# lab-incert/peba1

Hardware: AMD Instinct MI355X
Metric: bootstrapped gates/sec (blind rotations/s) over the PEBA1 match path, and end-to-end match ms (higher is better)
Workload: dtype u32

## Files before the change

### include/tfhe_hip.h

```cpp
#ifndef TFHE_HIP_H
#define TFHE_HIP_H

#include <stdio.h>

#include "tfhe/tfhe_core.h"

#ifdef __cplusplus
extern "C" {
#endif

enum TfheHipGate {
    TFHE_HIP_NAND = 0, TFHE_HIP_OR, TFHE_HIP_AND, TFHE_HIP_NOR, TFHE_HIP_XOR, TFHE_HIP_XNOR,
    TFHE_HIP_ANDNY, TFHE_HIP_ANDYN, TFHE_HIP_ORNY, TFHE_HIP_ORYN
};

const char *tfhe_hip_last_error(void);
void tfhe_hip_clear_error(void);

int tfhe_hip_set_device(int device);
int tfhe_hip_get_device(void);
int tfhe_hip_device_pci_bus_id(char *out, int len);

TFheGateBootstrappingParameterSet *tfhe_hip_new_parameters(
    int32_t n, int32_t N, int32_t k, int32_t l, int32_t Bgbit, int32_t ks_t, int32_t ks_basebit,
    double ks_stdev, double bk_stdev, double max_stdev);
TFheGateBootstrappingParameterSet *tfhe_hip_new_p2048_parameters(void);

TFheGateBootstrappingSecretKeySet *tfhe_hip_new_secret_keyset_seeded(
    const TFheGateBootstrappingParameterSet *params, uint64_t seed);
TFheGateBootstrappingSecretKeySet *tfhe_hip_new_secret_keyset_seeded_host(
    const TFheGateBootstrappingParameterSet *params, uint64_t seed);
void tfhe_hip_set_encrypt_seed(uint64_t seed);
int tfhe_hip_randomness_is_seeded(void);
void tfhe_hip_test_chacha20_block(const uint32_t *key8, uint64_t counter, const uint32_t *nonce2, uint32_t *out16);

const int32_t *tfhe_hip_key_lwe(const TFheGateBootstrappingSecretKeySet *key, int64_t *count);
const int32_t *tfhe_hip_key_tlwe(const TFheGateBootstrappingSecretKeySet *key, int64_t *count);
const Torus32 *tfhe_hip_key_bk(const TFheGateBootstrappingCloudKeySet *cloud, int64_t *count);
const Torus32 *tfhe_hip_key_ksk(const TFheGateBootstrappingCloudKeySet *cloud, int64_t *count);

int32_t tfhe_hip_sample_words(const TFheGateBootstrappingParameterSet *params);
int tfhe_hip_export_samples(const LweSample *samples, int32_t count,
                            const TFheGateBootstrappingParameterSet *params, Torus32 *out_words);
int tfhe_hip_import_samples(LweSample *samples, int32_t count,
                            const TFheGateBootstrappingParameterSet *params, const Torus32 *in_words);
int tfhe_hip_export_samples_device(const LweSample *samples, int32_t count,
                                   const TFheGateBootstrappingParameterSet *params, void *device_words);
int tfhe_hip_import_samples_device(LweSample *samples, int32_t count,
                                   const TFheGateBootstrappingParameterSet *params, const void *device_words);
int tfhe_hip_export_samples_device_async(const LweSample *samples, int32_t count,
                                         const TFheGateBootstrappingParameterSet *params, void *device_words);
int tfhe_hip_import_samples_device_async(LweSample *samples, int32_t count,
                                         const TFheGateBootstrappingParameterSet *params, const void *device_words);
void *tfhe_hip_stream(void);
int tfhe_hip_sync_samples(const LweSample *samples, int32_t count);

void tfhe_hip_set_deferred(int on);
int tfhe_hip_get_deferred(void);
int tfhe_hip_flush(void);
int tfhe_hip_flush_async(void);
int tfhe_hip_wait(void);

#define TFHE_HIP_EXIT_DEADLINE 86
int tfhe_hip_stream_sync(void);
int tfhe_hip_wait_event(void *hip_event, const char *what);
void tfhe_hip_set_diag_label(const char *label);

int tfhe_hip_gate_batch(int gate, LweSample *result, const LweSample *a, const LweSample *b,
                        int32_t count, const TFheGateBootstrappingCloudKeySet *bk);

enum TfheHipGate3 { TFHE_HIP_MAJ3 = 0, TFHE_HIP_XOR3, TFHE_HIP_XNOR3 };
void tfhe_hip_gate3(int gate, int negate_mask, LweSample *result, const LweSample *a, const LweSample *b,
                    const LweSample *c, const TFheGateBootstrappingCloudKeySet *bk);
int tfhe_hip_gate3_batch(int gate, int negate_mask, LweSample *result, const LweSample *a, const LweSample *b,
                         const LweSample *c, int32_t count, const TFheGateBootstrappingCloudKeySet *bk);

typedef struct TfheHipLut TfheHipLut;
TfheHipLut *tfhe_hip_new_lut(const TFheGateBootstrappingParameterSet *params, const Torus32 *v);
TfheHipLut *tfhe_hip_new_lut_constant(const TFheGateBootstrappingParameterSet *params, Torus32 mu);
TfheHipLut *tfhe_hip_new_lut_from_table(const TFheGateBootstrappingParameterSet *params, const Torus32 *values, int32_t slots);
void tfhe_hip_delete_lut(TfheHipLut *lut);
const Torus32 *tfhe_hip_lut_words(const TfheHipLut *lut, int32_t *count);
void tfhe_hip_lut_bootstrap(const TfheHipLut *lut, LweSample *result, int32_t nin, const LweSample *const *in,
                            const int32_t *coef, Torus32 c0, const TFheGateBootstrappingCloudKeySet *bk);
int tfhe_hip_lut_bootstrap_batch(const TfheHipLut *lut, LweSample *result, int32_t nin, const LweSample *const *in,
                                 const int32_t *coef, Torus32 c0, int32_t count, const TFheGateBootstrappingCloudKeySet *bk);

typedef struct TfheHipLutMulti TfheHipLutMulti;
TfheHipLutMulti *tfhe_hip_new_lut_multi(const TfheHipLut *lut, int32_t nout, const int32_t *ntaps, const int32_t *tap_index,
                                        const int32_t *tap_weight, const Torus32 *out_c0);
TfheHipLutMulti *tfhe_hip_new_lut_multi_from_tables(const TFheGateBootstrappingParameterSet *params, Torus32 step, int32_t slots,
                                                    int32_t nout, const int32_t *levels );
void tfhe_hip_delete_lut_multi(TfheHipLutMulti *mo);
int32_t tfhe_hip_lut_multi_nout(const TfheHipLutMulti *mo);
int32_t tfhe_hip_lut_multi_output(const TfheHipLutMulti *mo, int32_t m, int32_t *tap_index, int32_t *tap_weight, Torus32 *out_c0);
const Torus32 *tfhe_hip_lut_multi_words(const TfheHipLutMulti *mo, int32_t *count);
void tfhe_hip_lut_bootstrap_multi(const TfheHipLutMulti *mo, LweSample *const *result , int32_t nin,
                                  const LweSample *const *in, const int32_t *coef, Torus32 c0,
                                  const TFheGateBootstrappingCloudKeySet *bk);
int tfhe_hip_lut_bootstrap_multi_batch(const TfheHipLutMulti *mo, LweSample *const *result , int32_t nin,
                                       const LweSample *const *in, const int32_t *coef, Torus32 c0, int32_t count,
                                       const TFheGateBootstrappingCloudKeySet *bk);

#define TFHE_HIP_LINEAR_MAX_IN 16
void tfhe_hip_linear(LweSample *result, int32_t nin, const LweSample *const *in, const int32_t *coef, Torus32 c0,
                     const TFheGateBootstrappingCloudKeySet *bk);
int tfhe_hip_linear_batch(LweSample *result, int32_t nin, const LweSample *const *in, const int32_t *coef, Torus32 c0,
                          int32_t count, const TFheGateBootstrappingCloudKeySet *bk);
void tfhe_hip_sym_encrypt_torus(LweSample *result, Torus32 mu, const TFheGateBootstrappingSecretKeySet *key);
Torus32 tfhe_hip_sym_phase(const LweSample *sample, const TFheGateBootstrappingSecretKeySet *key);

int tfhe_hip_set_tuning(const char *name, int64_t value);

typedef struct TfheHipStats {
    uint64_t blind_rotates;
    uint64_t keyswitches;
    uint64_t linear_ops;
    uint64_t levels;
    uint64_t flushes;
    uint64_t br_launches;
    double   ms_blind_rotate;
    double   ms_keyswitch;
    double   ms_flush_wall;
    double   ms_blind_rotate_busy;
    uint64_t reused_gates;
    uint64_t br8_launches;
    uint64_t br8_rotations;
    double   ms_blind_rotate8;
    uint64_t clk_shader_cycles;
    uint64_t clk_ref_ticks;
    uint64_t dead_gates;
    uint64_t folded_gates;
    uint64_t br_wide4_launches;
    uint64_t br_split_launches;
    uint64_t br_wave8_launches;
    uint64_t br_wave2_launches;
    uint64_t br_tables0_launches;
    uint64_t br_tables1_launches;
    uint64_t br_tables2_launches;
    uint64_t lut_rotations;
    uint64_t multi_rotations;
    uint64_t multi_outputs;
    uint64_t lincomb_ops;
    uint64_t lincomb_launches;
    uint64_t ks_pergate_launches;
    uint64_t ks_strip_launches;
    uint64_t ks_index_launches;
    uint64_t unpacked_samples;
    uint64_t unpack_launches;
} TfheHipStats;
void tfhe_hip_get_stats(TfheHipStats *out);
void tfhe_hip_reset_stats(void);
typedef struct TfheHipExpandStats {
    uint64_t expanded_keys;
    uint64_t expand_launches;
} TfheHipExpandStats;
void tfhe_hip_get_expand_stats(TfheHipExpandStats *out);
typedef struct TfheHipSeededStats {
    uint64_t expanded_packing_keys;
    uint64_t packing_expand_launches;
    uint64_t seeded_unpacked_samples;
    uint64_t seeded_unpack_launches;
} TfheHipSeededStats;
void tfhe_hip_get_seeded_stats(TfheHipSeededStats *out);
typedef struct TfheHipSeededLweStats {
    uint64_t seeded_imported_samples;
    uint64_t seeded_import_launches;
} TfheHipSeededLweStats;
void tfhe_hip_get_seeded_lwe_stats(TfheHipSeededLweStats *out);
void tfhe_hip_set_kernel_timing(int on);
int tfhe_hip_last_flush_keys(void);
int tfhe_hip_set_batch_keys(int on);

int tfhe_hip_test_form_admissible(int form, int32_t N, int32_t l, int32_t Bgbit, int tables);

int tfhe_hip_test_stage_place(int64_t pos, int64_t capacity, int32_t outstanding, int64_t bytes, int64_t *out4);

void tfhe_hip_test_set_alloc_cap(int64_t bytes);

int tfhe_hip_test_schedule(const int32_t *ops5, int32_t count, int32_t unit, int32_t balance, int32_t *levels_out);
int tfhe_hip_test_level_plan(const int32_t *ops5, const int32_t *op_keys, int32_t count, int32_t nkeys, int32_t unit,
                             int32_t balance, int32_t *levels_out, int32_t *sizes6, int32_t *rot_off, int32_t *ks_off,
                             int32_t *rot_koff, int32_t *ks_koff, int32_t *rot_key, int32_t *rots6, int32_t *kss4);
int tfhe_hip_test_level_plan3(const int32_t *ops5, const int32_t *op_keys, int32_t count, int32_t nkeys, int32_t unit,
                              int32_t balance, int32_t *levels_out, int32_t *sizes6, int32_t *rot_off, int32_t *ks_off,
                              int32_t *rot_koff, int32_t *ks_koff, int32_t *rot_key, int32_t *rots8, int32_t *kss4);
int tfhe_hip_test_level_plan_lut(const int32_t *ops10, const int32_t *op_keys, int32_t count, int32_t nkeys, int32_t unit,
                                 int32_t balance, int32_t reuse, int32_t *levels_out, int32_t *shared_with, int32_t *sizes6,
                                 int32_t *rot_off, int32_t *ks_off, int32_t *rot_koff, int32_t *ks_koff, int32_t *rot_key,
                                 int32_t *rots9, int32_t *kss4);
int tfhe_hip_test_level_plan_multi(const int32_t *ops16, const int32_t *op_keys, int32_t count, int32_t nkeys, int32_t unit,
                                   int32_t balance, int32_t reuse, const int32_t *dead_slots, int32_t ndead,
                                   int32_t *levels_out, int32_t *shared_with, int32_t *sizes6, int32_t *rot_off, int32_t *ks_off,
                                   int32_t *rot_koff, int32_t *ks_koff, int32_t *rot_key, int32_t *rots10, int32_t *kss4);
int tfhe_hip_test_level_plan_lin(const int32_t *ops16, const int32_t *op_keys, int32_t count, int32_t nkeys, int32_t unit,
                                 int32_t balance, int32_t reuse, const int32_t *dead_slots, int32_t ndead,
                                 const int32_t *lin_terms2, int32_t nterms, int32_t *levels_out, int32_t *ranks_out,
                                 int32_t *shared_with, int32_t *sizes6, int32_t *rot_off, int32_t *ks_off, int32_t *rot_koff,
                                 int32_t *ks_koff, int32_t *rot_key, int32_t *rots10, int32_t *kss4, int32_t *lin_sizes2,
                                 int32_t *lin_level_off, int32_t *lin_launch_off, int32_t *lin_launch_rank, int32_t *lins35);
int tfhe_hip_test_level_plan_full(const int32_t *ops16, const int32_t *op_keys, int32_t count, int32_t nkeys, int32_t unit,
                                  int32_t balance, int32_t reuse, const int32_t *dead_slots, int32_t ndead,
                                  const int32_t *lin_terms2, int32_t nterms, int32_t *levels_out, int32_t *ranks_out,
                                  int32_t *shared_with, int32_t *sizes6, int32_t *rot_off, int32_t *ks_off, int32_t *rot_koff,
                                  int32_t *ks_koff, int32_t *rot_key, int32_t *rots10, int32_t *kss4, int32_t *lin_sizes2,
                                  int32_t *lin_level_off, int32_t *lin_launch_off, int32_t *lin_launch_rank, int32_t *lins35,
                                  int32_t *not_off, int32_t *nots2);
int tfhe_hip_test_level_slack(const int32_t *ops5, int32_t count, int32_t unit, int32_t level_slack, const int32_t *cost_widths,
                              const double *cost_us, int32_t ncost, int32_t period, int32_t *levels_out, int32_t *widths_out,
                              double *cost_out2);
int tfhe_hip_test_level_cost(int32_t n, int32_t N, int32_t k, int32_t l, int32_t Bgbit, int32_t ks_t, int32_t ks_basebit,
                             int32_t cu_count, int32_t width, double *us_out);
int tfhe_hip_test_set_level_cost(const int32_t *cost_widths, const double *cost_us, int32_t ncost);
int tfhe_hip_last_level_slack(double *out4);
int tfhe_hip_test_br_plan(int32_t N, int32_t l, int32_t Bgbit, const int32_t *tunings4, int32_t cu_count, int32_t count,
                          int32_t flags, int32_t *out3);
int tfhe_hip_test_ks_plan(int32_t n, int32_t N, int32_t k, int32_t ks_t, int32_t ks_basebit, const int32_t *tunings5,
                          int32_t cu_count, int32_t count, int64_t *out6);
int tfhe_hip_test_ks_plan_form(int32_t n, int32_t N, int32_t k, int32_t ks_t, int32_t ks_basebit, const int32_t *tunings5,
                               int32_t cu_count, int32_t count, int64_t *out7);
int tfhe_hip_test_wg_times(const TFheGateBootstrappingCloudKeySet *bk, int32_t width, uint64_t *times4, double *launch_ms);

typedef struct TfheHipPackingKey TfheHipPackingKey;
TfheHipPackingKey *tfhe_hip_new_packing_key(const TFheGateBootstrappingSecretKeySet *secret, int32_t pk_t, int32_t pk_basebit);
TfheHipPackingKey *tfhe_hip_new_packing_key_seeded(const TFheGateBootstrappingSecretKeySet *secret, int32_t pk_t,
                                                   int32_t pk_basebit, uint64_t seed);
TfheHipPackingKey *tfhe_hip_new_packing_key_from_words(const TFheGateBootstrappingParameterSet *params, int32_t pk_t,
                                                       int32_t pk_basebit, const Torus32 *words);
void tfhe_hip_delete_packing_key(TfheHipPackingKey *key);
const Torus32 *tfhe_hip_packing_key_words(const TfheHipPackingKey *key, int64_t *count);
int tfhe_hip_packing_key_decomposition(const TfheHipPackingKey *key, int32_t *pk_t, int32_t *pk_basebit);
int tfhe_hip_pack_samples(const TfheHipPackingKey *key, const LweSample *samples, int32_t count,
                          const TFheGateBootstrappingCloudKeySet *bk, Torus32 *out_words);
int tfhe_hip_pack_samples_device(const TfheHipPackingKey *key, const LweSample *samples, int32_t count,
                                 const TFheGateBootstrappingCloudKeySet *bk, void *device_words);
int tfhe_hip_packed_phase(const TFheGateBootstrappingSecretKeySet *secret, const Torus32 *words, Torus32 *out_phases);
int tfhe_hip_packed_decrypt_bits(const TFheGateBootstrappingSecretKeySet *secret, const Torus32 *words, int32_t count,
                                 int32_t *out_bits);
int tfhe_hip_test_pack_bounds(int32_t N, int32_t rows, int32_t basebit);

int tfhe_hip_ring_encrypt(const TFheGateBootstrappingSecretKeySet *secret, const Torus32 *mu, Torus32 *out_words);
int tfhe_hip_ring_encrypt_seeded(const TFheGateBootstrappingSecretKeySet *secret, const Torus32 *mu, Torus32 *out_words,
                                 uint64_t seed);
int tfhe_hip_ring_encrypt_bits(const TFheGateBootstrappingSecretKeySet *secret, const int32_t *bits, int32_t count,
                               Torus32 *out_words);
int tfhe_hip_ring_encrypt_bits_seeded(const TFheGateBootstrappingSecretKeySet *secret, const int32_t *bits, int32_t count,
                                      Torus32 *out_words, uint64_t seed);
int tfhe_hip_unpack_samples(const TFheGateBootstrappingCloudKeySet *bk, const Torus32 *ring_words, int32_t nring,
                            const int32_t *index, int32_t count, LweSample *result);
int tfhe_hip_unpack_samples_scattered(const TFheGateBootstrappingCloudKeySet *bk, const Torus32 *ring_words, int32_t nring,
                                      const int32_t *index, int32_t count, LweSample *const *result);
int tfhe_hip_unpack_samples_device(const TFheGateBootstrappingCloudKeySet *bk, const void *device_ring_words, int32_t nring,
                                   const int32_t *index, int32_t count, LweSample *result);

typedef struct TfheHipCompressedCloudKey TfheHipCompressedCloudKey;
TfheHipCompressedCloudKey *tfhe_hip_new_compressed_cloud_key(const TFheGateBootstrappingSecretKeySet *secret);
TfheHipCompressedCloudKey *tfhe_hip_new_compressed_cloud_key_seeded(const TFheGateBootstrappingSecretKeySet *secret,
                                                                    uint64_t noise_seed, const uint32_t *mask_seed10);
TfheHipCompressedCloudKey *tfhe_hip_new_compressed_cloud_key_from_words(const TFheGateBootstrappingParameterSet *params,
                                                                        const uint32_t *mask_seed10, const Torus32 *bk_body,
                                                                        const Torus32 *ksk_body);
void tfhe_hip_delete_compressed_cloud_key(TfheHipCompressedCloudKey *key);
const uint32_t *tfhe_hip_compressed_key_seed(const TfheHipCompressedCloudKey *key);
const Torus32 *tfhe_hip_compressed_key_bk_body(const TfheHipCompressedCloudKey *key, int64_t *count);
const Torus32 *tfhe_hip_compressed_key_ksk_body(const TfheHipCompressedCloudKey *key, int64_t *count);
int64_t tfhe_hip_compressed_key_bytes(const TfheHipCompressedCloudKey *key);
TFheGateBootstrappingCloudKeySet *tfhe_hip_expand_cloud_key_host(const TfheHipCompressedCloudKey *key);
TFheGateBootstrappingCloudKeySet *tfhe_hip_expand_cloud_key(const TfheHipCompressedCloudKey *key);
void tfhe_hip_export_compressed_cloud_key_toFile(FILE *F, const TfheHipCompressedCloudKey *key);
TfheHipCompressedCloudKey *tfhe_hip_new_compressed_cloud_key_fromFile(FILE *F);
int tfhe_hip_kernel_expand_masks(const uint32_t *mask_seed10, int64_t first_word, int32_t count, uint32_t *out);
int64_t tfhe_hip_test_key_image(const TFheGateBootstrappingCloudKeySet *cloud, int which, Torus32 *out, int64_t capacity);
double tfhe_hip_last_expand_ms(void);

typedef struct TfheHipCompressedPackingKey TfheHipCompressedPackingKey;
TfheHipCompressedPackingKey *tfhe_hip_new_compressed_packing_key(const TFheGateBootstrappingSecretKeySet *secret, int32_t pk_t,
                                                                 int32_t pk_basebit);
TfheHipCompressedPackingKey *tfhe_hip_new_compressed_packing_key_seeded(const TFheGateBootstrappingSecretKeySet *secret,
                                                                        int32_t pk_t, int32_t pk_basebit, uint64_t noise_seed,
                                                                        const uint32_t *mask_seed10);
TfheHipCompressedPackingKey *tfhe_hip_new_compressed_packing_key_from_words(const TFheGateBootstrappingParameterSet *params,
                                                                            int32_t pk_t, int32_t pk_basebit,
                                                                            const uint32_t *mask_seed10, const Torus32 *body);
void tfhe_hip_delete_compressed_packing_key(TfheHipCompressedPackingKey *key);
const uint32_t *tfhe_hip_compressed_packing_key_seed(const TfheHipCompressedPackingKey *key);
const Torus32 *tfhe_hip_compressed_packing_key_body(const TfheHipCompressedPackingKey *key, int64_t *count);
int tfhe_hip_compressed_packing_key_decomposition(const TfheHipCompressedPackingKey *key, int32_t *pk_t, int32_t *pk_basebit);
int64_t tfhe_hip_compressed_packing_key_bytes(const TfheHipCompressedPackingKey *key);
TfheHipPackingKey *tfhe_hip_expand_packing_key_host(const TfheHipCompressedPackingKey *key);
TfheHipPackingKey *tfhe_hip_expand_packing_key(const TfheHipCompressedPackingKey *key);
void tfhe_hip_export_compressed_packing_key_toFile(FILE *F, const TfheHipCompressedPackingKey *key);
TfheHipCompressedPackingKey *tfhe_hip_new_compressed_packing_key_fromFile(FILE *F);
#define TFHE_HIP_RING_COMPRESSED_WORDS(N) (10 + (N))
int tfhe_hip_ring_encrypt_compressed(const TFheGateBootstrappingSecretKeySet *secret, const Torus32 *mu, Torus32 *out_words);
int tfhe_hip_ring_encrypt_compressed_seeded(const TFheGateBootstrappingSecretKeySet *secret, const Torus32 *mu,
                                            Torus32 *out_words, const uint32_t *mask_seed10, uint64_t noise_seed);
int tfhe_hip_ring_encrypt_bits_compressed(const TFheGateBootstrappingSecretKeySet *secret, const int32_t *bits, int32_t count,
                                          Torus32 *out_words);
int tfhe_hip_ring_encrypt_bits_compressed_seeded(const TFheGateBootstrappingSecretKeySet *secret, const int32_t *bits,
                                                 int32_t count, Torus32 *out_words, const uint32_t *mask_seed10,
                                                 uint64_t noise_seed);
int tfhe_hip_ring_expand_host(const Torus32 *compressed_words, int32_t N, Torus32 *out_words);
int tfhe_hip_unpack_samples_seeded(const TFheGateBootstrappingCloudKeySet *bk, const Torus32 *compressed_words, int32_t nring,
                                   const int32_t *index, int32_t count, LweSample *result);
int tfhe_hip_unpack_samples_seeded_scattered(const TFheGateBootstrappingCloudKeySet *bk, const Torus32 *compressed_words,
                                             int32_t nring, const int32_t *index, int32_t count, LweSample *const *result);
int tfhe_hip_unpack_samples_seeded_device(const TFheGateBootstrappingCloudKeySet *bk, const void *device_compressed_words,
                                          int32_t nring, const int32_t *index, int32_t count, LweSample *result);
int64_t tfhe_hip_test_pack_image(const TfheHipPackingKey *key, const TFheGateBootstrappingCloudKeySet *bk, Torus32 *out,
                                 int64_t capacity);
int64_t tfhe_hip_test_extract_rows(Torus32 *out, int64_t capacity);

#define TFHE_HIP_LWE_COMPRESSED_WORDS(count) (10 + (count))
#define TFHE_HIP_LWE_RECORD_MAX (1 << 20)
int tfhe_hip_sym_encrypt_bits_compressed(const TFheGateBootstrappingSecretKeySet *secret, const int32_t *bits, int32_t count,
                                         Torus32 *out_words);
int tfhe_hip_sym_encrypt_bits_compressed_seeded(const TFheGateBootstrappingSecretKeySet *secret, const int32_t *bits, int32_t count,
                                                Torus32 *out_words, const uint32_t *mask_seed10, uint64_t noise_seed);
int tfhe_hip_sym_encrypt_torus_compressed(const TFheGateBootstrappingSecretKeySet *secret, const Torus32 *mu, int32_t count,
                                          Torus32 *out_words);
int tfhe_hip_sym_encrypt_torus_compressed_seeded(const TFheGateBootstrappingSecretKeySet *secret, const Torus32 *mu, int32_t count,
                                                 Torus32 *out_words, const uint32_t *mask_seed10, uint64_t noise_seed);
int tfhe_hip_lwe_expand_host(const Torus32 *compressed_words, int32_t n, int32_t record_count, const int32_t *index, int32_t count,
                             Torus32 *out_words);
int tfhe_hip_import_samples_seeded(const TFheGateBootstrappingParameterSet *params, const Torus32 *compressed_words,
                                   int32_t record_count, const int32_t *index, int32_t count, LweSample *result);
int tfhe_hip_import_samples_seeded_scattered(const TFheGateBootstrappingParameterSet *params, const Torus32 *compressed_words,
                                             int32_t record_count, const int32_t *index, int32_t count, LweSample *const *result);
int tfhe_hip_import_samples_seeded_device(const TFheGateBootstrappingParameterSet *params, const void *device_compressed_words,
                                          int32_t record_count, const int32_t *index, int32_t count, LweSample *result);
int tfhe_hip_kernel_lwe_expand(const TFheGateBootstrappingParameterSet *params, const Torus32 *compressed_words, int32_t record_count,
                               const int32_t *index, int32_t count, Torus32 *out_words);
int64_t tfhe_hip_test_expand_slots(Torus32 *out, int64_t capacity);

typedef struct TfheHipSelector TfheHipSelector;
int64_t tfhe_hip_tgsw_words(const TFheGateBootstrappingParameterSet *params);
int tfhe_hip_tgsw_encrypt_bits(const TFheGateBootstrappingSecretKeySet *secret, const int32_t *bits, int32_t count,
                               Torus32 *out_words);
int tfhe_hip_tgsw_encrypt_bits_seeded(const TFheGateBootstrappingSecretKeySet *secret, const int32_t *bits, int32_t count,
                                      Torus32 *out_words, uint64_t seed);
TfheHipSelector *tfhe_hip_new_selector(const TFheGateBootstrappingParameterSet *params, const Torus32 *words, int32_t nbits);
void tfhe_hip_delete_selector(TfheHipSelector *selector);
int32_t tfhe_hip_selector_bits(const TfheHipSelector *selector);
int tfhe_hip_ring_select(const TfheHipSelector *selector, const Torus32 *ring_words, int32_t M, Torus32 *out_ring_words);
int tfhe_hip_ring_select_device(const TfheHipSelector *selector, const void *device_ring_words, int32_t M, void *device_out);
double tfhe_hip_last_select_ms(void);
int tfhe_hip_kernel_ring_cmux(const TfheHipSelector *selector, int32_t bit_index, const Torus32 *d1_words, const Torus32 *d0_words,
                              int32_t count, Torus32 *out_words);
int tfhe_hip_test_select_bounds(int32_t N, int32_t l, int32_t Bgbit);

int tfhe_hip_kernel_negacyclic(const TFheGateBootstrappingCloudKeySet *bk, const int32_t *ip,
                               const Torus32 *tp, Torus32 *res, int32_t count);
int tfhe_hip_kernel_bootstrap_woks(const TFheGateBootstrappingCloudKeySet *bk, const Torus32 *lin,
                                   int32_t count, Torus32 *u_out, Torus32 *acc_out);
int tfhe_hip_kernel_lut_bootstrap_woks(const TFheGateBootstrappingCloudKeySet *bk, const Torus32 *lin, int32_t count,
                                       const int32_t *lut_index, const Torus32 *polys, int32_t npolys, Torus32 *u_out,
                                       Torus32 *acc_out);
#define TFHE_HIP_EXTRACT_SPEC_WORDS 73
int tfhe_hip_kernel_lut_bootstrap_multi_woks(const TFheGateBootstrappingCloudKeySet *bk, const Torus32 *lin, int32_t count,
                                             const int32_t *lut_index, const Torus32 *polys, int32_t npolys,
                                             const int32_t *spec_index, const int32_t *specs, int32_t nspecs, Torus32 *u_out,
                                             Torus32 *acc_out);
int tfhe_hip_kernel_keyswitch(const TFheGateBootstrappingCloudKeySet *bk, const Torus32 *u,
                              int32_t count, Torus32 *out);
int tfhe_hip_kernel_pack(const TfheHipPackingKey *key, const TFheGateBootstrappingCloudKeySet *bk, const Torus32 *sample_words,
                         int32_t count, int32_t idx_per_wg, Torus32 *out_words);
int tfhe_hip_kernel_ring_extract(const TFheGateBootstrappingCloudKeySet *bk, const Torus32 *ring_words, int32_t nring,
                                 const int32_t *index, int32_t count, Torus32 *u_out);
int tfhe_hip_kernel_ring_extract_seeded(const TFheGateBootstrappingCloudKeySet *bk, const Torus32 *compressed_words, int32_t nring,
                                        const int32_t *index, int32_t count, Torus32 *u_out);

#ifdef __cplusplus
}
#endif
#endif
```

### peba1_amd/api.py

```python
import ctypes as C

import numpy as np

from . import lib as _l

GATE_CODES = {"NAND": 0, "OR": 1, "AND": 2, "NOR": 3, "XOR": 4, "XNOR": 5,
              "ANDNY": 6, "ANDYN": 7, "ORNY": 8, "ORYN": 9}
GATE3_CODES = {"MAJ3": 0, "XOR3": 1, "XNOR3": 2}
GATE3_LIN = {"MAJ3": 1, "XOR3": -2, "XNOR3": 2}


def _i32p(a):
    assert a.dtype == np.int32 and a.flags["C_CONTIGUOUS"]
    return a.ctypes.data_as(_l.I32P)


def last_error():
    return _l.load().tfhe_hip_last_error().decode()


class _CFile:
    _libc = None

    def __init__(self, path, mode):
# ... 86 lines not shown
            self.ptr = None

    def _arr(self, f, owner):
        cnt = C.c_int64()
        p = f(owner, C.byref(cnt))
        return np.ctypeslib.as_array(p, shape=(cnt.value,))

    def lwe_key(self):
        return self._arr(_l.load().tfhe_hip_key_lwe, self.ptr)

    def tlwe_key(self):
        return self._arr(_l.load().tfhe_hip_key_tlwe, self.ptr)

    def bk(self):
        return self._arr(_l.load().tfhe_hip_key_bk, self.cloud)

    def ksk(self):
        return self._arr(_l.load().tfhe_hip_key_ksk, self.cloud)


class CloudKeySet(SecretKeySet):

    def __init__(self, ptr):
        self.ptr = None
        self.cloud = ptr
        self.params = ParameterSet(_ptr=C.cast(ptr.contents.params, _l.PS))

    @classmethod
    def load(cls, path):
        with _CFile(path, "rb") as fp:
            ptr = _l.load().new_tfheGateBootstrappingCloudKeySet_fromFile(fp)
        if not ptr:
            raise ValueError("cannot load a cloud keyset from %s: %s" % (path, last_error()))
        return cls(ptr)

    def save(self, path):
        with _CFile(path, "wb") as fp:
            _l.load().export_tfheGateBootstrappingCloudKeySet_toFile(fp, self.cloud)

    save_cloud = save

    def close(self):
        if self.cloud:
            _l.load().delete_gate_bootstrapping_cloud_keyset(self.cloud)
            self.cloud = None

    def lwe_key(self):
        raise TypeError("a cloud keyset holds no secret key")

    tlwe_key = lwe_key


class CompressedCloudKey:

    def __init__(self, ptr, params):
        if not ptr:
            raise RuntimeError("compressed cloud key refused: " + last_error())
        self.ptr, self.params = ptr, params

    @classmethod
    def generate(cls, secret):
        return cls(_l.load().tfhe_hip_new_compressed_cloud_key(secret.ptr), secret.params)

    @classmethod
    def generate_seeded(cls, secret, noise_seed, mask_seed):
        seed = np.ascontiguousarray(mask_seed, dtype=np.uint32).reshape(10)
        return cls(_l.load().tfhe_hip_new_compressed_cloud_key_seeded(secret.ptr, noise_seed, seed.ctypes.data_as(_l.U32P)),
                   secret.params)

    @classmethod
    def from_words(cls, params, mask_seed, bk_body, ksk_body):
        seed = np.ascontiguousarray(mask_seed, dtype=np.uint32).reshape(10)
        base = (1 << params.ks_basebit) - 1
        bk = np.ascontiguousarray(bk_body, dtype=np.int32).reshape(params.n * (params.k + 1) * params.l * params.N)
        ksk = np.ascontiguousarray(ksk_body, dtype=np.int32).reshape(params.k * params.N * params.ks_t * base)
        return cls(_l.load().tfhe_hip_new_compressed_cloud_key_from_words(params.ptr, seed.ctypes.data_as(_l.U32P), _i32p(bk),
                                                                          _i32p(ksk)), params)

    def seed(self):
        return np.ctypeslib.as_array(_l.load().tfhe_hip_compressed_key_seed(self.ptr), shape=(10,)).copy()

    def _body(self, f):
        cnt = C.c_int64()
        p = f(self.ptr, C.byref(cnt))
        return np.ctypeslib.as_array(p, shape=(cnt.value,))

    def bk_body(self):
        return self._body(_l.load().tfhe_hip_compressed_key_bk_body)

    def ksk_body(self):
        return self._body(_l.load().tfhe_hip_compressed_key_ksk_body)

    @property
    def nbytes(self):
        return int(_l.load().tfhe_hip_compressed_key_bytes(self.ptr))

    def expand(self):
        ptr = _l.load().tfhe_hip_expand_cloud_key(self.ptr)
        if not ptr:
            raise RuntimeError("expand failed: " + last_error())
        return CloudKeySet(ptr)

    def expand_host(self):
        ptr = _l.load().tfhe_hip_expand_cloud_key_host(self.ptr)
        if not ptr:
            raise RuntimeError("expand_host failed: " + last_error())
        return CloudKeySet(ptr)

    def save(self, path):
        with _CFile(path, "wb") as fp:
            _l.load().tfhe_hip_export_compressed_cloud_key_toFile(fp, self.ptr)

    @classmethod
    def load(cls, path):
        with _CFile(path, "rb") as fp:
            ptr = _l.load().tfhe_hip_new_compressed_cloud_key_fromFile(fp)
        if not ptr:
            raise ValueError("cannot load a compressed cloud key from %s: %s" % (path, last_error()))
        return cls(ptr, None)

    def close(self):
        if self.ptr:
            _l.load().tfhe_hip_delete_compressed_cloud_key(self.ptr)
            self.ptr = None

    def __del__(self):
        try:
            self.close()
        except Exception:
            pass


def kernel_expand_masks(mask_seed, first_word, count):
    seed = np.ascontiguousarray(mask_seed, dtype=np.uint32).reshape(10)
    out = np.zeros(count, dtype=np.uint32)
    rc = _l.load().tfhe_hip_kernel_expand_masks(seed.ctypes.data_as(_l.U32P), first_word, count, out.ctypes.data_as(_l.U32P))
    if rc != 0:
        raise RuntimeError(last_error())
    return out


def key_image(key, which):
    L = _l.load()
    L.tfhe_hip_clear_error()
    words = L.tfhe_hip_test_key_image(key.cloud, which, None, 0)
    if words < 0:
        raise RuntimeError(last_error())
    out = np.zeros(words, dtype=np.int32)
    if L.tfhe_hip_test_key_image(key.cloud, which, _i32p(out), words) != words:
        raise RuntimeError(last_error())
    return out


def expand_stats():
    s = _l.ExpandStats()
    _l.load().tfhe_hip_get_expand_stats(C.byref(s))
    return {f: getattr(s, f) for f in _l.EXPAND_STATS_FIELDS}


class CiphertextArray:

    def __init__(self, params, count):
        self.params, self.count = params, count
        self.ptr = _l.load().new_gate_bootstrapping_ciphertext_array(count, params.ptr)

    def close(self):
        if self.ptr:
            _l.load().delete_gate_bootstrapping_ciphertext_array(self.count, self.ptr)
            self.ptr = None

    def __del__(self):
        try:
            self.close()
        except Exception:
            pass

    def at(self, i):
        return C.cast(C.addressof(self.ptr.contents) + i * C.sizeof(_l.LweSample), _l.LS)

    def encrypt(self, bits, key):
        L = _l.load()
        for i, b in enumerate(bits):
            L.bootsSymEncrypt(self.at(i), int(b), key.ptr)
        return self

    def decrypt(self, key):
        L = _l.load()
        return np.array([L.bootsSymDecrypt(self.at(i), key.ptr) for i in range(self.count)], dtype=np.int32)

    def save(self, path):
        L = _l.load()
        with _CFile(path, "wb") as fp:
            for i in range(self.count):
                L.export_gate_bootstrapping_ciphertext_toFile(fp, self.at(i), self.params.ptr)

    def load(self, path):
        L = _l.load()
        with _CFile(path, "rb") as fp:
            for i in range(self.count):
                L.tfhe_hip_clear_error()
                L.import_gate_bootstrapping_ciphertext_fromFile(fp, self.at(i), self.params.ptr)
                if last_error():
                    raise ValueError("cannot load ciphertext %d from %s: %s" % (i, path, last_error()))
        return self

    def words(self):
        out = np.zeros((self.count, self.params.words), dtype=np.int32)
        rc = _l.load().tfhe_hip_export_samples(self.ptr, self.count, self.params.ptr, _i32p(out))
        if rc != 0:
            raise RuntimeError(last_error())
        return out

    def set_words(self, w):
        w = np.ascontiguousarray(w, dtype=np.int32).reshape(self.count, self.params.words)
        rc = _l.load().tfhe_hip_import_samples(self.ptr, self.count, self.params.ptr, _i32p(w))
        if rc != 0:
            raise RuntimeError(last_error())
        return self


def gate_batch(name, result, a, b, key):
    rc = _l.load().tfhe_hip_gate_batch(GATE_CODES[name], result.ptr, a.ptr, b.ptr, result.count, key.cloud)
    if rc != 0:
        raise RuntimeError(last_error())


def gate3(name, result, a, b, c, key, negate_mask=0):
    _l.load().tfhe_hip_gate3(GATE3_CODES[name], int(negate_mask), result, a, b, c, key.cloud)


def gate3_batch(name, result, a, b, c, key, negate_mask=0):
    rc = _l.load().tfhe_hip_gate3_batch(GATE3_CODES[name], int(negate_mask), result.ptr, a.ptr, b.ptr, c.ptr, result.count,
                                        key.cloud)
    if rc != 0:
        raise RuntimeError(last_error())


class Lut:

    def __init__(self, params, words):
        w = np.ascontiguousarray(words, dtype=np.int32)
        if w.shape != (params.N,):
            raise ValueError("a LUT of this parameter set holds %d words" % params.N)
        self._take(params, _l.load().tfhe_hip_new_lut(params.ptr, _i32p(w)))

    def _take(self, params, ptr):
        self.params, self.ptr = params, ptr
        if not ptr:
            raise ValueError("LUT rejected: " + last_error())

    @classmethod
    def constant(cls, params, mu):
        self = cls.__new__(cls)
        self._take(params, _l.load().tfhe_hip_new_lut_constant(params.ptr, int(mu)))
        return self

    @classmethod
    def from_table(cls, params, values):
        v = np.ascontiguousarray(values, dtype=np.int32)
        self = cls.__new__(cls)
        self._take(params, _l.load().tfhe_hip_new_lut_from_table(params.ptr, _i32p(v), len(v)))
        return self

    def words(self):
        cnt = C.c_int32()
        p = _l.load().tfhe_hip_lut_words(self.ptr, C.byref(cnt))
        return np.ctypeslib.as_array(p, shape=(cnt.value,)).copy()

    def close(self):
        if self.ptr:
            _l.load().tfhe_hip_delete_lut(self.ptr)
            self.ptr = None

    def __del__(self):
        try:
            self.close()
        except Exception:
            pass


def lut_bootstrap(lut, result, inputs, coefs, c0, key):
    n = len(inputs)
    ins = (_l.LS * max(n, 1))(*inputs)
    cf = np.ascontiguousarray(coefs, dtype=np.int32)
    assert len(cf) == n
    _l.load().tfhe_hip_lut_bootstrap(lut.ptr if lut is not None else None, result, n, ins, _i32p(cf), int(c0), key.cloud)


def lut_bootstrap_batch(lut, result, inputs, coefs, c0, key):
    n = len(inputs)
    ins = (_l.LS * max(n, 1))(*[a.ptr for a in inputs])
    cf = np.ascontiguousarray(coefs, dtype=np.int32)
    assert len(cf) == n
    rc = _l.load().tfhe_hip_lut_bootstrap_batch(lut.ptr if lut is not None else None, result.ptr, n, ins, _i32p(cf), int(c0),
                                                result.count, key.cloud)
    if rc != 0:
        raise RuntimeError(last_error())


class LutMulti:

    def __init__(self, lut, outputs):
        ntaps = np.array([len(t) for t, _ in outputs], dtype=np.int32)
        idx = np.array([i for t, _ in outputs for i, _ in t] or [0], dtype=np.int32)
        wgt = np.array([w for t, _ in outputs for _, w in t] or [0], dtype=np.int32)
        c0 = np.array([_wrap32(c) for _, c in outputs] or [0], dtype=np.int32)
# ... 577 lines not shown


LINEAR_MAX_IN = 16


def linear(result, inputs, coefs, c0, key):
    n = len(inputs)
    ins = (_l.LS * max(n, 1))(*inputs)
    cf = np.ascontiguousarray([_wrap32(c) for c in coefs] or [0], dtype=np.int32)
    assert len(coefs) == n
    _l.load().tfhe_hip_linear(result, n, ins, _i32p(cf), _wrap32(c0), key.cloud)


def linear_batch(result, inputs, coefs, c0, key):
    n = len(inputs)
    ins = (_l.LS * max(n, 1))(*[a.ptr for a in inputs])
    cf = np.ascontiguousarray([_wrap32(c) for c in coefs] or [0], dtype=np.int32)
    assert len(coefs) == n
    rc = _l.load().tfhe_hip_linear_batch(result.ptr, n, ins, _i32p(cf), _wrap32(c0), result.count, key.cloud)
    if rc != 0:
        raise RuntimeError(last_error())


def encrypt_torus(sample, mu, key):
    _l.load().tfhe_hip_sym_encrypt_torus(sample, _wrap32(mu), key.ptr)


def phase(sample, key):
    return int(_l.load().tfhe_hip_sym_phase(sample, key.ptr))


def set_deferred(on):
    _l.load().tfhe_hip_set_deferred(1 if on else 0)


def get_deferred():
    return bool(_l.load().tfhe_hip_get_deferred())


def flush():
    return _l.load().tfhe_hip_flush()


def flush_async():
    return _l.load().tfhe_hip_flush_async()


def wait():
    return _l.load().tfhe_hip_wait()


def set_tuning(name, value):
    if _l.load().tfhe_hip_set_tuning(name.encode(), int(value)) != 0:
        raise ValueError(last_error())


def stats():
    s = _l.StatsWhole()
    _l.load().tfhe_hip_get_stats(C.byref(s))
    return {f: getattr(s, f) for f in _l.STATS_FIELDS}


def unpack_stats():
    s = _l.StatsWhole()
    _l.load().tfhe_hip_get_stats(C.byref(s))
    return {f: getattr(s, f) for f in _l.UNPACK_STATS_FIELDS}


def last_flush_keys():
    return _l.load().tfhe_hip_last_flush_keys()


def reset_stats():
    _l.load().tfhe_hip_reset_stats()


def kernel_negacyclic(key, ip, tp):
    ip = np.ascontiguousarray(ip, dtype=np.int32)
    tp = np.ascontiguousarray(tp, dtype=np.int32)
    res = np.zeros_like(tp)
    rc = _l.load().tfhe_hip_kernel_negacyclic(key.cloud, _i32p(ip), _i32p(tp), _i32p(res), ip.shape[0])
    if rc != 0:
        raise RuntimeError(last_error())
    return res


def kernel_bootstrap_woks(key, lin, want_acc=False):
    p = key.params
    lin = np.ascontiguousarray(lin, dtype=np.int32).reshape(-1, p.words)
    u = np.zeros((lin.shape[0], p.k * p.N + 1), dtype=np.int32)
    acc = np.zeros((lin.shape[0], (p.k + 1) * p.N), dtype=np.int32) if want_acc else None
    rc = _l.load().tfhe_hip_kernel_bootstrap_woks(key.cloud, _i32p(lin), lin.shape[0], _i32p(u),
                                                  _i32p(acc) if want_acc else None)
    if rc != 0:
        raise RuntimeError(last_error())
    return (u, acc) if want_acc else u


def kernel_lut_bootstrap_woks(key, lin, lut_index, polys, want_acc=False):
    p = key.params
    lin = np.ascontiguousarray(lin, dtype=np.int32).reshape(-1, p.words)
    idx = np.ascontiguousarray(lut_index, dtype=np.int32).reshape(lin.shape[0])
    polys = np.ascontiguousarray(polys, dtype=np.int32).reshape(-1, p.N)
    u = np.zeros((lin.shape[0], p.k * p.N + 1), dtype=np.int32)
    acc = np.zeros((lin.shape[0], (p.k + 1) * p.N), dtype=np.int32) if want_acc else None
    rc = _l.load().tfhe_hip_kernel_lut_bootstrap_woks(key.cloud, _i32p(lin), lin.shape[0], _i32p(idx), _i32p(polys),
                                                      polys.shape[0], _i32p(u), _i32p(acc) if want_acc else None)
    if rc != 0:
        raise RuntimeError(last_error())
    return (u, acc) if want_acc else u


EXTRACT_SPEC_WORDS = 73


def pack_extract_specs(specs):
    out = np.zeros((len(specs), EXTRACT_SPEC_WORDS), dtype=np.int32)
    for rec, outputs in zip(out, specs):
        rec[0] = len(outputs)
        for m, (taps, c0) in enumerate(outputs):
            rec[1 + m] = len(taps)
            rec[5 + m] = _wrap32(c0)
            for t, (i, w) in enumerate(taps):
                rec[9 + 8 * m + t] = i
                rec[41 + 8 * m + t] = w
    return out


def kernel_lut_bootstrap_multi_woks(key, lin, lut_index, polys, spec_index, specs, want_acc=False):
    p = key.params
    lin = np.ascontiguousarray(lin, dtype=np.int32).reshape(-1, p.words)
    idx = np.ascontiguousarray(lut_index, dtype=np.int32).reshape(lin.shape[0])
    sidx = np.ascontiguousarray(spec_index, dtype=np.int32).reshape(lin.shape[0])
    polys = np.ascontiguousarray(polys, dtype=np.int32).reshape(-1, p.N)
    recs = pack_extract_specs(specs)
    u = np.zeros((lin.shape[0], 4, p.k * p.N + 1), dtype=np.int32)
    acc = np.zeros((lin.shape[0], (p.k + 1) * p.N), dtype=np.int32) if want_acc else None
    rc = _l.load().tfhe_hip_kernel_lut_bootstrap_multi_woks(key.cloud, _i32p(lin), lin.shape[0], _i32p(idx), _i32p(polys),
                                                            polys.shape[0], _i32p(sidx), _i32p(recs), recs.shape[0], _i32p(u),
                                                            _i32p(acc) if want_acc else None)
    if rc != 0:
        raise RuntimeError(last_error())
    return (u, acc) if want_acc else u


def kernel_keyswitch(key, u):
    p = key.params
    u = np.ascontiguousarray(u, dtype=np.int32).reshape(-1, p.k * p.N + 1)
    out = np.zeros((u.shape[0], p.words), dtype=np.int32)
    rc = _l.load().tfhe_hip_kernel_keyswitch(key.cloud, _i32p(u), u.shape[0], _i32p(out))
    if rc != 0:
        raise RuntimeError(last_error())
    return out
```

### peba1_amd/csrc/engine.cpp

```cpp
#include "engine.hpp"

#include <algorithm>
#include <utility>
#include <vector>
#include <chrono>
#include <ctime>
#include <unistd.h>
#include <cstdio>
#include <cstdlib>
#include <cstring>
#include <mutex>

#include "br_forms.hpp"
#include "ntt_field.hpp"

namespace tfhe_hip {

static std::string g_last_error;
static std::mutex g_err_mtx;

void set_error(const std::string &msg) {
    std::lock_guard<std::mutex> g(g_err_mtx);
    g_last_error = msg;
}
// ... 332 lines not shown
    img->dp = make_dev_params(p);
    fill_form_ok(img->form_ok, p.N, p.l, p.Bgbit);
    uint32_t scale[2];
    const std::vector<uint32_t> tw = make_twiddles(p.N, scale);
    const size_t bk_words = p.bk_words();
    const int base = 1 << p.ks_basebit, stride = p.ct_stride();
    const size_t rows = (size_t)p.k * p.N * p.ks_t;
    int32_t *raw = nullptr;
    try {
        img->tw_bytes = tw.size() * 4;
        img->tw = static_cast<uint32_t *>(recoverable_alloc(img->tw_bytes, "the twiddle tables of a key"));
        img->bk_img_bytes = bk_words * 2 * 4;
        img->bk_img = static_cast<uint32_t *>(recoverable_alloc(img->bk_img_bytes, "the bootstrapping-key image"));
        img->ksk_bytes = (rows * (base - 1) + 1) * (size_t)stride * 4;
        img->ksk = static_cast<int32_t *>(recoverable_alloc(img->ksk_bytes, "the key-switching key"));
        raw = static_cast<int32_t *>(recoverable_alloc(bk_words * 4, "the staging copy of the bootstrapping key"));
    } catch (const ApiError &) {
        recoverable_free(img->tw, img->tw_bytes);
        recoverable_free(img->bk_img, img->bk_img_bytes);
        recoverable_free(img->ksk, img->ksk_bytes);
        delete img;
        throw;
    }
    hip_check(hipMemcpy(img->tw, tw.data(), tw.size() * 4, hipMemcpyHostToDevice), "upload twiddles");

    hip_check(hipMemcpy(raw, ck.bk.data(), bk_words * 4, hipMemcpyHostToDevice), "upload bk");
    launch_bk_transform(stream_, img->dp, raw, img->bk_img, img->tw, p.n * p.kpl(), p.k + 1, scale);
    hip_check(hipGetLastError(), "bk_transform launch");
    sync_stream("bk_transform");
    recoverable_free(raw, bk_words * 4);

    std::vector<int32_t> compact((rows * (base - 1) + 1) * stride, 0);
    for (size_t r = 0; r < rows; ++r)
        for (int v = 1; v < base; ++v)
            std::memcpy(&compact[(r * (base - 1) + (v - 1)) * stride], &ck.ksk[(r * base + v) * (size_t)(p.n + 1)],
                        (size_t)(p.n + 1) * 4);
    hip_check(hipMemcpy(img->ksk, compact.data(), compact.size() * 4, hipMemcpyHostToDevice), "upload ksk");

    img->key.bk_img = img->bk_img;
    img->key.ksk = img->ksk;
    img->key.ksk_zero = img->ksk + rows * (base - 1) * stride;
    img->key.tw = img->tw;
    return img;
}

DeviceKeyImage *Engine::upload_compressed_key(const TfheHipCloudKey &ck) {
    ENGINE_DEVICE_SCOPE();
    ensure_init();
    const Params &p = ck.p;
    if (const char *why = unsupported_reason(p)) api_fail(why);
    auto *img = new DeviceKeyImage();
    img->dp = make_dev_params(p);
    fill_form_ok(img->form_ok, p.N, p.l, p.Bgbit);
    uint32_t scale[2];
    const std::vector<uint32_t> tw = make_twiddles(p.N, scale);
    const size_t bk_words = p.bk_words(), bk_body = p.bk_body_words() * 4, ksk_body = p.ksk_body_words() * 4;
    const int stride = p.ct_stride();
    const size_t rows = p.ksk_body_words();
    int32_t *raw = nullptr, *dbk = nullptr, *dksk = nullptr;
    try {
        img->tw_bytes = tw.size() * 4;
        img->tw = static_cast<uint32_t *>(recoverable_alloc(img->tw_bytes, "the twiddle tables of a key"));
        img->bk_img_bytes = bk_words * 2 * 4;
        img->bk_img = static_cast<uint32_t *>(recoverable_alloc(img->bk_img_bytes, "the bootstrapping-key image"));
        img->ksk_bytes = (rows + 1) * (size_t)stride * 4;
        img->ksk = static_cast<int32_t *>(recoverable_alloc(img->ksk_bytes, "the key-switching key"));
        raw = static_cast<int32_t *>(recoverable_alloc(bk_words * 4, "the staging copy of the bootstrapping key"));
        dbk = static_cast<int32_t *>(recoverable_alloc(bk_body, "the bodies of a compressed bootstrapping key"));
        dksk = static_cast<int32_t *>(recoverable_alloc(ksk_body, "the bodies of a compressed key-switching key"));
    } catch (const ApiError &) {
        recoverable_free(dbk, bk_body);
        recoverable_free(raw, bk_words * 4);
        recoverable_free(img->tw, img->tw_bytes);
        recoverable_free(img->bk_img, img->bk_img_bytes);
        recoverable_free(img->ksk, img->ksk_bytes);
        delete img;
        throw;
    }
    hip_check(hipMemcpy(img->tw, tw.data(), tw.size() * 4, hipMemcpyHostToDevice), "upload twiddles");
    hip_check(hipMemcpy(dbk, ck.bk_body.data(), bk_body, hipMemcpyHostToDevice), "upload bk bodies");
    hip_check(hipMemcpy(dksk, ck.ksk_body.data(), ksk_body, hipMemcpyHostToDevice), "upload ksk bodies");

    ExpandSeed seed;
    std::memcpy(seed.key, ck.mask_seed.data(), sizeof seed.key);
    seed.nonce[0] = ck.mask_seed[8]; seed.nonce[1] = ck.mask_seed[9];
    hipEvent_t e0 = nullptr, e1 = nullptr;
    if (kernel_timing) {
        hip_check(hipEventCreate(&e0), "expand event");
        hip_check(hipEventCreate(&e1), "expand event");
        hip_check(hipEventRecord(e0, stream_), "expand event");
    }
    const ExpandBkArgs ba{seed, p.n * p.kpl(), p.k, p.N, dbk, raw};
    const ExpandKskArgs ka{seed, (uint64_t)(p.bk_mask_words() / 8), (int64_t)rows, p.n, stride, dksk, img->ksk};
    if (!launch_expand_bk(stream_, ba) || !launch_expand_ksk(stream_, ka)) fatal("expand: arguments outside what the kernels were built for");
    hip_check(hipGetLastError(), "expand launch");
    if (kernel_timing) hip_check(hipEventRecord(e1, stream_), "expand event");
    hip_check(hipMemsetAsync(img->ksk + rows * stride, 0, (size_t)stride * 4, stream_), "clear the zero row");
    launch_bk_transform(stream_, img->dp, raw, img->bk_img, img->tw, p.n * p.kpl(), p.k + 1, scale);
    hip_check(hipGetLastError(), "bk_transform launch");
    sync_stream("key expansion");
    if (kernel_timing) {
        float ms = 0.f;
        hip_check(hipEventElapsedTime(&ms, e0, e1), "expand event");
        last_expand_ms = ms;
        (void)hipEventDestroy(e0);
        (void)hipEventDestroy(e1);
    }
    recoverable_free(raw, bk_words * 4);
    recoverable_free(dbk, bk_body);
    recoverable_free(dksk, ksk_body);
    ++expand_stats.expanded_keys;
    expand_stats.expand_launches += 2;

    img->key.bk_img = img->bk_img;
    img->key.ksk = img->ksk;
    img->key.ksk_zero = img->ksk + rows * stride;
    img->key.tw = img->tw;
    return img;
}

void Engine::run_expand_masks(const uint32_t seed10[10], int64_t first_word, int count, uint32_t *out) {
    ENGINE_DEVICE_SCOPE();
    ensure_init();
    wait_flight();
    ExpandSeed seed;
    std::memcpy(seed.key, seed10, sizeof seed.key);
    seed.nonce[0] = seed10[8]; seed.nonce[1] = seed10[9];
    uint32_t *d = scratch_as<uint32_t>(S_EXPAND_WORDS, (size_t)count);
    if (!launch_expand_masks(stream_, seed, first_word, count, d)) api_fail("expand_masks: arguments outside what the kernel was built for");
    hip_check(hipGetLastError(), "expand_masks launch");
    ++expand_stats.expand_launches;
    d2h(out, d, (size_t)count, "download stream words");
    sync_stream("expand_masks");
}

size_t Engine::read_key_image(const DeviceKeyImage *img, int which, Torus32 *out, size_t capacity) {
    ENGINE_DEVICE_SCOPE();
    const size_t words = (which == 0 ? img->bk_img_bytes : img->ksk_bytes) / 4;
    if (!out || capacity < words) return words;
    wait_flight();
    const void *src = which == 0 ? static_cast<const void *>(img->bk_img) : static_cast<const void *>(img->ksk);
    hip_check(hipMemcpyAsync(out, src, words * 4, hipMemcpyDeviceToHost, stream_), "download key image");
    sync_stream("key image");
    return words;
}

void Engine::free_key(DeviceKeyImage *img) {
    ENGINE_DEVICE_SCOPE();
    if (!img) return;
    if (inited_) sync_stream("sync before key free");
    recoverable_free(img->bk_img, img->bk_img_bytes);
    recoverable_free(img->ksk, img->ksk_bytes);
    recoverable_free(img->tw, img->tw_bytes);
    delete img;
}

static std::vector<int32_t> pad_rows(const int32_t *src, size_t rows, size_t words, size_t stride) {
    std::vector<int32_t> padded(rows * stride, 0);
    for (size_t r = 0; r < rows; ++r) std::memcpy(&padded[r * stride], src + r * words, words * 4);
    return padded;
}
static void unpad_rows(int32_t *dst, const int32_t *src, size_t rows, size_t words, size_t stride) {
    for (size_t r = 0; r < rows; ++r) std::memcpy(dst + r * words, src + r * stride, words * 4);
}

namespace {
struct DeviceTable {
    const size_t entry;
    const char *const grow_what, *const sync_what;
    char *dev = nullptr;
    size_t cap = 0, used = 0;
    std::vector<int32_t> free;
    int32_t add(const void *src) {
        if (free.empty() && used == cap) {
            const size_t fresh_cap = cap ? cap * 2 : 16;
            char *fresh = static_cast<char *>(recoverable_alloc(fresh_cap * entry, grow_what));
            if (dev) {
                Engine::get().sync_stream(sync_what);
                hip_check(hipDeviceSynchronize(), sync_what);
                hip_check(hipMemcpy(fresh, dev, cap * entry, hipMemcpyDeviceToDevice), grow_what);
                recoverable_free(dev, cap * entry);
            }
            dev = fresh;
            cap = fresh_cap;
        }
        int32_t index;
        if (!free.empty()) { index = free.back(); free.pop_back(); }
        else index = (int32_t)used++;
        hip_check(hipMemcpy(dev + (size_t)index * entry, src, entry, hipMemcpyHostToDevice), "upload a table entry");
        return index;
    }
    void release(int32_t index) { if (index >= 0 && (size_t)index < used) free.push_back(index); }
};
DeviceTable g_luts{(size_t)LUT_STRIDE * sizeof(int32_t), "growing the table of test polynomials", "sync before LUT table growth"};
DeviceTable g_specs{sizeof(ExtractSpec), "growing the table of extract specs", "sync before spec table growth"};
}

int32_t Engine::lut_add(const Torus32 *words, int n_ring) {
    ENGINE_DEVICE_SCOPE();
    ensure_init();
    if (n_ring < 1 || n_ring > LUT_STRIDE) api_fail("a test polynomial of more than " + std::to_string(LUT_STRIDE) + " words");
    return g_luts.add(pad_rows(words, 1, (size_t)n_ring, LUT_STRIDE).data());
}
void Engine::lut_free(int32_t index) { g_luts.release(index); }

int32_t Engine::spec_add(const ExtractSpec &xs) {
    ENGINE_DEVICE_SCOPE();
    ensure_init();
    if (g_specs.free.empty() && g_specs.used == g_specs.cap && g_specs.cap > (size_t)XS_ENTRY_MASK / 2) api_fail("too many extract specs");
    const int32_t index = g_specs.add(&xs);
    if (spec_nout_.size() <= (size_t)index) spec_nout_.resize((size_t)index + 1, 0);
    spec_nout_[(size_t)index] = xs.nout;
    return index;
}
void Engine::spec_free(int32_t index) { g_specs.release(index); }

SlotPool *Engine::find_pool(const Params &p) const {
    for (SlotPool *pl : pools_)
        if (pl->ct_stride() == p.ct_stride() && pl->ct_words() == p.ct_words()) return pl;
    return nullptr;
}

SlotPool *Engine::pool_for(const Params &p) {
    ENGINE_DEVICE_SCOPE();
    ensure_init();
    if (SlotPool *pl = find_pool(p)) return pl;
    size_t cap = 1u << 22;
    if (const char *env = std::getenv("TFHE_HIP_POOL_SLOTS")) cap = (size_t)std::atoll(env);
    if (cap < 8 || cap > MAX_POOL_SLOTS) {
        set_error("TFHE_HIP_POOL_SLOTS out of range [8, 2^29]; clamped");
        cap = cap < 8 ? 8 : MAX_POOL_SLOTS;
    }
    auto *pl = new SlotPool(p.ct_words(), p.ct_stride(), cap);
    std::vector<Torus32> z(p.n, 0);
    pl->const_slot[0] = pl->alloc();
    write_slot(pl, pl->const_slot[0], z.data(), -(1 << 29));
    pl->const_slot[1] = pl->alloc();
    write_slot(pl, pl->const_slot[1], z.data(), 1 << 29);
    pools_.push_back(pl);
    return pl;
}

void Engine::write_slot(SlotPool *pool, int32_t slot, const Torus32 *a, Torus32 b) {
    ENGINE_DEVICE_SCOPE();
    sync_io();
    std::vector<int32_t> tmp(pool->ct_stride(), 0);
    std::memcpy(tmp.data(), a, (size_t)(pool->ct_words() - 1) * 4);
    tmp[pool->ct_words() - 1] = b;
    hip_check(hipMemcpy(pool->data() + (size_t)slot * pool->ct_stride(), tmp.data(), tmp.size() * 4, hipMemcpyHostToDevice),
              "write_slot");
}

void Engine::read_slot(SlotPool *pool, int32_t slot, Torus32 *a, Torus32 *b) {
    ENGINE_DEVICE_SCOPE();
    wait_flight();
    std::vector<int32_t> tmp(pool->ct_stride());
    d2h(tmp.data(), pool->data() + (size_t)slot * pool->ct_stride(), tmp.size(), "read_slot");
    sync_stream("read_slot");
    std::memcpy(a, tmp.data(), (size_t)(pool->ct_words() - 1) * 4);
    *b = tmp[pool->ct_words() - 1];
}

void Engine::write_slots_packed(SlotPool *pool, const int32_t *slots, int count, const Torus32 *words, bool on_device, bool wait) {
    ENGINE_DEVICE_SCOPE();
    if (count <= 0) return;
    if (count > MAX_PACKED_SAMPLES) api_fail("too many samples in one packed transfer");
    const size_t nwords = (size_t)count * pool->ct_words();
    int32_t *dslots = scratch_as<int32_t>(S_SLOTS, (size_t)count);
    h2d_staged(dslots, slots, (size_t)count, "upload slot list");
    const int32_t *src = on_device ? words : scratch_upload(S_WORDS, words, nwords, "upload packed words");
    launch_scatter_slots(stream_, pool->data(), pool->ct_stride(), pool->ct_words(), dslots, count, src);
    finish(wait || !on_device, "scatter slots");
}

void Engine::read_slots_packed(SlotPool *pool, const int32_t *slots, int count, Torus32 *words, bool on_device, bool wait) {
    ENGINE_DEVICE_SCOPE();
    if (count <= 0) return;
    if (count > MAX_PACKED_SAMPLES) api_fail("too many samples in one packed transfer");
    const size_t nwords = (size_t)count * pool->ct_words();
    int32_t *dslots = scratch_as<int32_t>(S_SLOTS, (size_t)count);
    h2d_staged(dslots, slots, (size_t)count, "upload slot list");
    int32_t *dst = on_device ? words : scratch_as<int32_t>(S_WORDS, nwords);
    launch_gather_slots(stream_, pool->data(), pool->ct_stride(), pool->ct_words(), dslots, count, dst);
    if (!on_device) d2h(words, dst, nwords, "download packed words");
    finish(wait || !on_device, "gather slots");
}

hipEvent_t Engine::next_timing_event() {
    if (timing_used_ == timing_events_.size()) {
        hipEvent_t e;
        hip_check(hipEventCreate(&e), "timing event");
        timing_events_.push_back(e);
    }
    return timing_events_[timing_used_++];
}

BrPlan Engine::plan_br_launch(const DeviceKeyImage *key, int count, bool acc_dump) const {
    const BrPlan plan = plan_br(key->form_ok, key->dp.N, key->dp.l, tunings, cu_count_, count, wg_times_dbg_ != nullptr, acc_dump);
    if (plan.form < 0) fatal("no admissible blind-rotate form (upload_key should have refused this key)");
    return plan;
}

void Engine::launch_br(const DeviceKeyImage *key, const BrPlan &plan, const BrLaunch &a) {
    ENGINE_DEVICE_SCOPE();
    const hipStream_t stream = a.stream ? a.stream : stream_;
    const int form = plan.form, head = a.count - plan.tail;
    if (a.mk_keys && form != BR_FORM_WIDE4 && form != BR_FORM_WAVE8) fatal("launch_br: no multi-key kernel for this form");
    if (plan.tail && (form != BR_FORM_WIDE4 || a.acc_dbg)) fatal("launch_br: a tail behind a launch that cannot be split");
    DevParams dp = key->dp;
    dp.digit_table = plan.tables;
    dp.luts = a.luts ? a.luts : reinterpret_cast<const int32_t *>(g_luts.dev);
    dp.specs = a.specs ? a.specs : reinterpret_cast<const ExtractSpec *>(g_specs.dev);
    auto note = [&](int f) {
        ++(f == BR_FORM_WIDE4 ? stats.br_wide4_launches : f == BR_FORM_SPLIT ? stats.br_split_launches
           : f == BR_FORM_WAVE8 ? stats.br_wave8_launches : stats.br_wave2_launches);
        const int ran = br_tables_run(f, dp.l, dp.Bgbit, plan.tables);
        ++(ran == 0 ? stats.br_tables0_launches : ran == 1 ? stats.br_tables1_launches : stats.br_tables2_launches);
    };
    if (kernel_timing) {
        if (!clock_acc_) {
            hip_check(hipMalloc(&clock_acc_, 2 * sizeof(unsigned long long)), "hipMalloc(clock sums)");
            hip_check(hipMemset(clock_acc_, 0, 2 * sizeof(unsigned long long)), "hipMemset(clock sums)");
        }
        dp.clock_acc = clock_acc_;
    }
    if (form == BR_FORM_WIDE4 || form == BR_FORM_WAVE8) dp.wg_times = wg_times_dbg_;
    note(form);
    if (form == BR_FORM_WAVE2) launch_blind_rotate2(stream, dp, key->key, a.pool, a.rots, a.count, a.u_buf, a.acc_dbg);
    else if (form == BR_FORM_SPLIT) launch_blind_rotate_split(stream, dp, key->key, a.pool, a.rots, a.count, a.u_buf, a.acc_dbg);
    else if (form == BR_FORM_WAVE8 && a.mk_keys) launch_blind_rotate8_mk(stream, dp, key->key, a.mk_keys, a.mk_rot_keys, a.pool, a.rots, a.count, a.u_buf);
    else if (form == BR_FORM_WAVE8) launch_blind_rotate8(stream, dp, key->key, a.pool, a.rots, a.count, a.u_buf, a.acc_dbg);
    else if (a.mk_keys) launch_blind_rotate4_mk(stream, dp, key->key, a.mk_keys, a.mk_rot_keys, a.pool, a.rots, head, a.u_buf);
    else launch_blind_rotate4(stream, dp, key->key, a.pool, a.rots, head, a.u_buf, a.acc_dbg);
    if (!plan.tail) return;
    if (a.mid) { *a.mid = next_timing_event(); hip_check(hipEventRecord(*a.mid, stream), "event"); }
    note(BR_FORM_WAVE8);
    if (a.mk_keys) launch_blind_rotate8_mk(stream, dp, key->key, a.mk_keys, a.mk_rot_keys + head, a.pool, a.rots + head, plan.tail, a.u_buf);
    else launch_blind_rotate8(stream, dp, key->key, a.pool, a.rots + head, plan.tail, a.u_buf, nullptr);
}

static KsShape ks_shape(const DevParams &dp) { return KsShape{dp.k * dp.N, dp.ks_t, dp.ks_basebit, dp.ct_stride}; }

void Engine::launch_ks(const DeviceKeyImage *key, const int32_t *u_buf, const KsDesc *descs, int count, int32_t *pool,
                       hipStream_t stream, bool presized) {
    ENGINE_DEVICE_SCOPE();
    if (count <= 0) return;
    if (!stream) stream = stream_;
    const DevParams &dp = key->dp;
    const KsShape shape = ks_shape(dp);
    const size_t bytes = ks_partial_bytes(tunings, cu_count_, count, shape);
    if (presized && bytes > (scratch_size_.size() > S_KS_PARTIAL ? scratch_size_[S_KS_PARTIAL] : 0))
        fatal("launch_ks: the key-switch partial sums were not sized by execute()");
    int32_t *partial = bytes ? static_cast<int32_t *>(scratch(S_KS_PARTIAL, bytes)) : nullptr;
    const KsPlan plan = plan_ks(tunings, count, shape);
    const int chunk = plan.form != KS_FORM_PERGATE ? KS_CHUNK : count;
    for (int done = 0; done < count; done += chunk) {
        const int cnt = std::min(chunk, count - done), splits = ks_splits(tunings, cu_count_, cnt, shape);
        const KsPlan part = done ? plan_ks(tunings, cnt, shape) : plan;
        ++(part.form == KS_FORM_INDEX ? stats.ks_index_launches : part.form == KS_FORM_STRIP ? stats.ks_strip_launches
                                                                                             : stats.ks_pergate_launches);
        if (!launch_keyswitch(stream, dp, key->key, u_buf, descs + done, cnt, pool, splits, splits > 1 ? partial : nullptr,
                              part.tile, part.form != KS_FORM_STRIP))
            fatal("launch_ks: the planned key-switch form has no kernel instantiation");
    }
}

Engine::FlushBuffers Engine::prepare_flush(const std::vector<const DeviceKeyImage *> &keys, LevelPlan &plan) {
    const DeviceKeyImage *key = keys.at(0);
    const int nkeys = plan.nkeys;
    if (nkeys < 1 || (size_t)nkeys != keys.size()) fatal("execute: the plan's key count differs from the flush's key list");
    for (const DeviceKeyImage *k : keys) {
        const DevParams &a = key->dp, &b = k->dp;
        if (a.n != b.n || a.N != b.N || a.k != b.k || a.l != b.l || a.Bgbit != b.Bgbit || a.ks_t != b.ks_t ||
            a.ks_basebit != b.ks_basebit)
            fatal("execute: the keys of a multi-key flush differ in a parameter that evaluation reads");
    }
    FlushBuffers fb{};
    fb.rots = scratch_as<RotDesc>(S_ROTS, plan.rots.size(), 16);
    fb.ks = scratch_as<KsDesc>(S_KS, plan.kss.size(), 16);
    fb.nots = scratch_as<NotDesc>(S_NOTS, plan.nots.size(), 16);
    if (!plan.lins.empty()) {
        if (plan.lin_level_off.size() != (size_t)plan.levels + 2 || plan.lin_launch_off.empty() ||
            (size_t)plan.lin_level_off.back() + 1 != plan.lin_launch_off.size() || (size_t)plan.lin_launch_off.back() != plan.lins.size())
            fatal("execute: the launch ranges of the linear combinations do not cover their descriptors");
        for (const LinDesc &d : plan.lins) {
            if (d.nin < 1 || d.nin > LIN_DESC_MAX_IN || d.dst_slot < 0) fatal("execute: a malformed linear combination");
            for (int t = 0; t < d.nin; ++t)
                if (d.slot[t] < 0 || d.slot[t] == d.dst_slot) fatal("execute: a linear combination reads a slot it may not");
        }
        fb.lins = scratch_as<LinDesc>(S_LINS, plan.lins.size());
    }
    fb.u_buf = scratch_as<int32_t>(S_EXTRACT, (size_t)(std::max(plan.max_rots, plan.max_extracts) + 1) * key->dp.u_stride);
    size_t partial = 0;
    const std::vector<int32_t> &ks_shares = nkeys == 1 ? plan.ks_off : plan.ks_koff;
    for (size_t sg = 0; sg + 1 < ks_shares.size(); ++sg)
        partial = std::max(partial, ks_partial_bytes(tunings, cu_count_, ks_shares[sg + 1] - ks_shares[sg], ks_shape(key->dp)));
    if (partial) (void)scratch(S_KS_PARTIAL, partial);
    if (nkeys > 1) {
        fb.keys = scratch_as<DevKey>(S_KEYS, (size_t)nkeys);
        fb.rot_keys = scratch_as<int32_t>(S_ROT_KEYS, plan.rot_key.size(), 16);
        plan.dev_keys.resize((size_t)nkeys);
        for (int k = 0; k < nkeys; ++k) plan.dev_keys[(size_t)k] = keys[(size_t)k]->key;
    }
    uint64_t lut_rots = 0, multi_rots = 0, multi_outs = 0;
    for (const RotDesc &rd : plan.rots) {
        if (rd.lut >= 0) {
            if ((size_t)rd.lut >= g_luts.used) fatal("execute: a rotation names a test polynomial the engine does not hold");
            ++lut_rots;
        }
        if (rd.spec >= 0) {
            if ((size_t)(rd.spec & XS_ENTRY_MASK) >= g_specs.used) fatal("execute: a rotation names an extract spec the engine does not hold");
            if (rd.u_index < 0 || rd.u_index + spec_nout_[(size_t)(rd.spec & XS_ENTRY_MASK)] > plan.max_extracts)
                fatal("execute: a multi-output rotation writes beyond the extract buffer");
            ++multi_rots;
            multi_outs += (uint64_t)__builtin_popcount((unsigned)(rd.spec >> XS_WANTED_SHIFT));
        }
    }
    stats.lut_rotations += lut_rots;
    stats.multi_rotations += multi_rots;
    stats.multi_outputs += multi_outs;
    return fb;
}

void Engine::upload_flush(const FlushBuffers &fb, LevelPlan &&plan_in) {
    flight_plan_ = std::move(plan_in);
    const LevelPlan &plan = flight_plan_;
    if (!plan.rots.empty()) h2d(fb.rots, plan.rots.data(), plan.rots.size(), "upload rots");
    if (!plan.kss.empty()) h2d(fb.ks, plan.kss.data(), plan.kss.size(), "upload ks");
    if (!plan.nots.empty()) h2d(fb.nots, plan.nots.data(), plan.nots.size(), "upload nots");
    if (!plan.lins.empty()) h2d(fb.lins, plan.lins.data(), plan.lins.size(), "upload lins");
    if (plan.nkeys > 1) {
        h2d(fb.keys, plan.dev_keys.data(), plan.dev_keys.size(), "upload keys");
        if (!plan.rot_key.empty()) h2d(fb.rot_keys, plan.rot_key.data(), plan.rot_key.size(), "upload rot keys");
    }
}

void Engine::run_level(const std::vector<const DeviceKeyImage *> &keys, SlotPool *pool, const FlushBuffers &fb, int L, hipEvent_t &shared_end) {
    const LevelPlan &plan = flight_plan_;
    const DeviceKeyImage *key = keys[0];
    const int nkeys = plan.nkeys;
    const size_t gg = L > 0 ? (size_t)(L - 1) : 0;
    const int nrot = L > 0 ? plan.rot_off[gg + 1] - plan.rot_off[gg] : 0;
    const int nks = L > 0 ? plan.ks_off[gg + 1] - plan.ks_off[gg] : 0;
    const int nnot = plan.not_off[(size_t)L + 1] - plan.not_off[(size_t)L];
    const int lin0 = plan.lins.empty() ? 0 : plan.lin_level_off[(size_t)L], lin1 = plan.lins.empty() ? 0 : plan.lin_level_off[(size_t)L + 1];
    if (nrot == 0 && nks == 0 && nnot == 0 && lin0 == lin1) return;
    Timed t{nullptr, nullptr, nullptr, false, nrot};
    if (kernel_timing) {
        if (shared_end) t.e0 = shared_end;
        else { t.e0 = next_timing_event(); hip_check(hipEventRecord(t.e0, stream_), "event"); }
        shared_end = nullptr;
    }
    if (nrot) {
        const BrPlan bp = plan_br_launch(key, nrot, false);
        int launches = 0;
        BrLaunch a{pool->data(), fb.rots + plan.rot_off[gg], nrot, fb.u_buf, nullptr, stream_};
        if (nkeys == 1 || bp.form == BR_FORM_WIDE4 || bp.form == BR_FORM_WAVE8) {
            a.mk_keys = fb.keys;
            a.mk_rot_keys = fb.keys ? fb.rot_keys + plan.rot_off[gg] : nullptr;
            a.mid = kernel_timing ? &t.em : nullptr;
            launch_br(key, bp, a);
            launches = bp.tail ? 2 : 1;
        } else {
            for (int k = 0; k < nkeys; ++k) {
                const size_t sg = gg * (size_t)nkeys + (size_t)k;
                a.rots = fb.rots + plan.rot_koff[sg];
                a.count = plan.rot_koff[sg + 1] - plan.rot_koff[sg];
                if (!a.count) continue;
                launch_br(keys[(size_t)k], bp, a);
                ++launches;
            }
        }
        t.wide8 = bp.form == BR_FORM_WAVE8;
        t.tail = bp.tail;
        stats.br_launches += (uint64_t)launches;
        if (t.wide8 || t.tail) { ++stats.br8_launches; stats.br8_rotations += (uint64_t)(t.wide8 ? nrot : t.tail); }
    }
    if (kernel_timing) { t.e1 = next_timing_event(); hip_check(hipEventRecord(t.e1, stream_), "event"); }
    for (int k = 0; k < nkeys && nks; ++k) {
        const size_t sg = gg * (size_t)nkeys + (size_t)k;
        const int32_t first = nkeys == 1 ? plan.ks_off[gg] : plan.ks_koff[sg];
        const int n = nkeys == 1 ? nks : plan.ks_koff[sg + 1] - first;
        if (n) launch_ks(keys[(size_t)k], fb.u_buf, fb.ks + first, n, pool->data(), stream_, true);
    }
    if (kernel_timing) {
        t.e2 = next_timing_event(); hip_check(hipEventRecord(t.e2, stream_), "event"); flight_timed_.push_back(t);
        if (nnot == 0 && lin0 == lin1) shared_end = t.e2;
    }
    launch_not(stream_, key->dp, fb.nots + plan.not_off[(size_t)L], nnot, pool->data());
    for (int j = lin0; j < lin1; ++j) {
        const int first = plan.lin_launch_off[(size_t)j], n = plan.lin_launch_off[(size_t)j + 1] - first;
        launch_linear(stream_, key->dp, fb.lins + first, n, pool->data());
        stats.linear_ops += (uint64_t)n;
        stats.lincomb_ops += (uint64_t)n;
        ++stats.lincomb_launches;
    }
    stats.blind_rotates += (uint64_t)nrot;
    stats.keyswitches += (uint64_t)nks;
    stats.linear_ops += (uint64_t)nnot;
}

void Engine::execute(const std::vector<const DeviceKeyImage *> &keys, SlotPool *pool, LevelPlan &&plan_in, bool wait) {
    ENGINE_DEVICE_SCOPE();
    wait_flight();
    flight_t0_ = std::chrono::steady_clock::now();
    const FlushBuffers fb = prepare_flush(keys, plan_in);
    upload_flush(fb, std::move(plan_in));
    const int levels = flight_plan_.levels;
    last_flush_keys = flight_plan_.nkeys;
    timing_used_ = 0;
    flight_timed_.clear();
    flight_base_ = nullptr;
    if (kernel_timing) {
        flight_base_ = next_timing_event();
        hip_check(hipEventRecord(flight_base_, stream_), "event");
        flight_timed_.reserve((size_t)levels + 1);
    }
    hipEvent_t shared_end = nullptr;
    for (int L = 0; L <= levels; ++L) run_level(keys, pool, fb, L, shared_end);
    if (const char *trace = std::getenv("TFHE_HIP_TRACE_LEVELS")) {
        if (FILE *f = std::fopen(trace, "a")) {
            std::fprintf(f, "flush levels=%d lanes=1\n", levels);
            for (int L = 1; L <= levels; ++L)
                std::fprintf(f, "%d 0 %d\n", L, flight_plan_.rot_off[(size_t)L] - flight_plan_.rot_off[(size_t)L - 1]);
            std::fclose(f);
        }
    }
    hip_check(hipGetLastError(), "kernel launch");
    flight_levels_ = levels;
    in_flight_ = true;
    if (wait) wait_flight();
}

void Engine::wait_flight() {
    ENGINE_DEVICE_SCOPE();
    if (!in_flight_) return;
    in_flight_ = false;
    const int levels = flight_levels_;
    std::vector<Timed> &timed = flight_timed_;
    hipEvent_t base = flight_base_;
    sync_stream("level execution");
    if (kernel_timing && base) {
        std::vector<std::pair<float, float>> br;
        br.reserve(timed.size());
        FILE *tf = nullptr;
        if (const char *trace = std::getenv("TFHE_HIP_TRACE_TIMES")) tf = std::fopen(trace, "a");
        static const auto trace_t0 = flight_t0_;
        if (tf) std::fprintf(tf, "flush levels=%d start_ms=%.3f\n", levels,
                             std::chrono::duration<double, std::milli>(flight_t0_ - trace_t0).count());
        for (const Timed &t : timed) {
            float a = 0, b = 0, c = 0;
            hip_check(hipEventElapsedTime(&a, base, t.e0), "elapsed");
            hip_check(hipEventElapsedTime(&b, base, t.e1), "elapsed");
            hip_check(hipEventElapsedTime(&c, base, t.e2), "elapsed");
            if (tf) std::fprintf(tf, "%d %.4f %.4f %.4f %d\n", t.nrot, a, b - a, c - b, t.wide8 ? 1 : 0);
            stats.ms_blind_rotate += b - a;
            if (t.wide8) stats.ms_blind_rotate8 += b - a;
            if (t.em) {
                float m = 0;
                hip_check(hipEventElapsedTime(&m, base, t.em), "elapsed");
                stats.ms_blind_rotate8 += b - m;
            }
            stats.ms_keyswitch += c - b;
            if (b > a) br.emplace_back(a, b);
        }
        std::sort(br.begin(), br.end());
        float cur_a = 0, cur_b = -1;
        for (const auto &iv : br) {
            if (cur_b < cur_a || iv.first > cur_b) {
                if (cur_b >= cur_a) stats.ms_blind_rotate_busy += cur_b - cur_a;
                cur_a = iv.first; cur_b = iv.second;
            } else {
                cur_b = std::max(cur_b, iv.second);
            }
        }
        if (cur_b >= cur_a) stats.ms_blind_rotate_busy += cur_b - cur_a;
        if (tf) {
            std::fprintf(tf, "wall_ms=%.3f\n", std::chrono::duration<double, std::milli>(std::chrono::steady_clock::now() - flight_t0_).count());
            std::fclose(tf);
        }
    }
    if (kernel_timing && clock_acc_) {
        unsigned long long sums[2] = {0, 0};
        hip_check(hipMemcpy(sums, clock_acc_, sizeof sums, hipMemcpyDeviceToHost), "read clock sums");
        hip_check(hipMemset(clock_acc_, 0, sizeof sums), "clear clock sums");
        stats.clk_shader_cycles += sums[0];
        stats.clk_ref_ticks += sums[1];
    }
    stats.levels += (uint64_t)levels;
    ++stats.flushes;
    stats.ms_flush_wall += std::chrono::duration<double, std::milli>(std::chrono::steady_clock::now() - flight_t0_).count();
    timed.clear();
    flight_plan_ = LevelPlan{};
}

void Engine::run_raw_rotations(const DeviceKeyImage *key, const Torus32 *lin, int count, const int32_t *lut_index,
                               const Torus32 *polys, int npolys, const int32_t *spec_index, const ExtractSpec *specs, int nspecs,
                               int out_rows, Torus32 *u_out, Torus32 *acc_out, const char *name) {
    ENGINE_DEVICE_SCOPE();
    wait_flight();
    const DevParams &dp = key->dp;
    const std::string who = std::string(name) + ": ";
    for (int c = 0; c < count; ++c) {
        if (lut_index && lut_index[c] >= npolys) api_fail(who + "a LUT index beyond the table");
        if (spec_index && spec_index[c] >= nspecs) api_fail(who + "a spec index beyond the table");
    }
    for (int t = 0; t < nspecs; ++t)
        if (const char *why = extract_spec_error(specs[t], dp.N)) api_fail(who + why);
    BrLaunch a{};
    const std::vector<int32_t> table = lut_index ? pad_rows(polys, (size_t)npolys, (size_t)dp.N, LUT_STRIDE) : std::vector<int32_t>();
    if (lut_index) a.luts = scratch_upload(S_RAW_LUTS, table.data(), table.size(), "upload LUTs");
    if (spec_index) a.specs = scratch_upload(S_RAW_SPECS, specs, (size_t)nspecs, "upload specs");
    const std::vector<int32_t> padded = pad_rows(lin, (size_t)count, (size_t)dp.n + 1, (size_t)dp.ct_stride);
    a.pool = scratch_upload(S_RAW_POOL, padded.data(), padded.size(), "upload lin");
    std::vector<RotDesc> rots(count);
    int32_t total = 0;
    for (int c = 0; c < count; ++c) {
        rots[c] = RotDesc{c, c, 1, 0, 0, total};
        if (lut_index && lut_index[c] >= 0) { rots[c].lut = lut_index[c]; ++stats.lut_rotations; }
        int nout = 1;
        if (spec_index && spec_index[c] >= 0) {
            nout = specs[spec_index[c]].nout;
            rots[c].spec = spec_index[c] | ((1 << nout) - 1) << XS_WANTED_SHIFT;
            ++stats.multi_rotations;
            stats.multi_outputs += (uint64_t)nout;
        }
        total += nout;
    }
    a.rots = scratch_upload(S_ROTS, rots.data(), rots.size(), "upload rots");
    a.count = count;
    a.u_buf = scratch_as<int32_t>(S_EXTRACT, (size_t)(total + 1) * dp.u_stride);
    a.acc_dbg = acc_out ? scratch_as<int32_t>(S_RAW_ACC, (size_t)count * 2 * dp.N) : nullptr;
    launch_br(key, plan_br_launch(key, count, a.acc_dbg != nullptr), a);
    hip_check(hipGetLastError(), "blind_rotate launch");
    std::vector<int32_t> ubuf((size_t)total * dp.u_stride);
    d2h(ubuf.data(), a.u_buf, ubuf.size(), "download u");
    if (acc_out) d2h(acc_out, a.acc_dbg, (size_t)count * 2 * dp.N, "download acc");
    sync_stream(name);
    const size_t uw = (size_t)dp.k * dp.N + 1;
    for (int c = 0; c < count; ++c) {
        const size_t nout = (size_t)((c + 1 < count ? rots[c + 1].u_index : total) - rots[c].u_index);
        unpad_rows(u_out + (size_t)c * out_rows * uw, &ubuf[(size_t)rots[c].u_index * dp.u_stride], nout, uw, (size_t)dp.u_stride);
    }
    stats.blind_rotates += (uint64_t)count;
}

void Engine::run_keyswitch(const DeviceKeyImage *key, const Torus32 *u, int count, Torus32 *out) {
    ENGINE_DEVICE_SCOPE();
    wait_flight();
    const DevParams &dp = key->dp;
    const std::vector<int32_t> padded = pad_rows(u, (size_t)count, (size_t)dp.k * dp.N + 1, (size_t)dp.u_stride);
    const int32_t *u_buf = scratch_upload(S_EXTRACT, padded.data(), padded.size(), "upload u");
    std::vector<KsDesc> ks(count);
    for (int c = 0; c < count; ++c) ks[c] = KsDesc{c, -1, 0, c};
    const KsDesc *dks = scratch_upload(S_KS, ks.data(), ks.size(), "upload ks");
    int32_t *dpool = scratch_as<int32_t>(S_RAW_POOL, (size_t)count * dp.ct_stride);
    launch_ks(key, u_buf, dks, count, dpool);
    hip_check(hipGetLastError(), "keyswitch launch");
    std::vector<int32_t> res((size_t)count * dp.ct_stride);
    d2h(res.data(), dpool, res.size(), "download ks");
    sync_stream("keyswitch");
    unpad_rows(out, res.data(), (size_t)count, (size_t)dp.n + 1, (size_t)dp.ct_stride);
    stats.keyswitches += (uint64_t)count;
}

double Engine::run_wg_times(const DeviceKeyImage *key, int width, unsigned long long *wg_times) {
    ENGINE_DEVICE_SCOPE();
    wait_flight();
    const DevParams &dp = key->dp;
    if (width <= 0 || !wg_times || dp.N != 1024) return -1.0;
    std::vector<int32_t> host((size_t)width * dp.ct_stride);
    uint64_t x = 0x9E3779B97F4A7C15ull;
    for (auto &w : host) { x ^= x << 13; x ^= x >> 7; x ^= x << 17; w = (int32_t)(x >> 16); }
    int32_t *pool = scratch_as<int32_t>(S_PROBE_POOL, (size_t)width * dp.ct_stride);
    hip_check(hipMemcpy(pool, host.data(), host.size() * 4, hipMemcpyHostToDevice), "probe pool");
    std::vector<RotDesc> rots(width);
    for (int i = 0; i < width; ++i) rots[i] = RotDesc{i, (i + 1) % width, 1, 1, -dp.mu, i};
    RotDesc *drots = scratch_as<RotDesc>(S_PROBE_ROTS, rots.size());
    hip_check(hipMemcpy(drots, rots.data(), rots.size() * sizeof(RotDesc), hipMemcpyHostToDevice), "probe rots");
    int32_t *ubuf = scratch_as<int32_t>(S_PROBE_EXTRACT, (size_t)(width + 1) * dp.u_stride);
    unsigned long long *dtimes = scratch_as<unsigned long long>(S_PROBE_TIMES, (size_t)4 * width);
    hipStream_t st;
    hip_check(hipStreamCreateWithFlags(&st, hipStreamNonBlocking), "probe stream");
    hipEvent_t e0, e1;
    hip_check(hipEventCreate(&e0), "probe event");
    hip_check(hipEventCreate(&e1), "probe event");
    int warm_count = 1, warm_width = width;
    if (const char *env = std::getenv("TFHE_HIP_PROBE_WARM")) std::sscanf(env, "%d:%d", &warm_count, &warm_width);
    warm_width = std::max(1, std::min(warm_width, width));
    BrLaunch a{pool, drots, warm_width, ubuf, nullptr, st};
    for (int w = 0; w < warm_count; ++w) launch_br(key, plan_br_launch(key, warm_width, false), a);
    hip_check(hipMemsetAsync(dtimes, 0, (size_t)4 * width * 8, st), "clear stamps");
    wg_times_dbg_ = dtimes;
    hip_check(hipEventRecord(e0, st), "probe event record");
    a.count = width;
    launch_br(key, plan_br_launch(key, width, false), a);
    hip_check(hipEventRecord(e1, st), "probe event record");
    hip_check(hipStreamSynchronize(st), "probe stamps");
    wg_times_dbg_ = nullptr;
    float ems = 0.f;
    hip_check(hipEventElapsedTime(&ems, e0, e1), "probe event time");
    (void)hipEventDestroy(e0); (void)hipEventDestroy(e1);
    hip_check(hipMemcpy(wg_times, dtimes, (size_t)4 * width * 8, hipMemcpyDeviceToHost), "probe stamps copy");
    hip_check(hipStreamDestroy(st), "probe stream destroy");
    for (int i = 0; i < width; ++i)
        if (wg_times[4 * i] == 0 || wg_times[4 * i + 1] == 0) return -1.0;
    return (double)ems;
}

void Engine::run_negacyclic(const DeviceKeyImage *key, const int32_t *ip, const Torus32 *tp, Torus32 *res, int count) {
    ENGINE_DEVICE_SCOPE();
    wait_flight();
    DevParams dp = key->dp;
    dp.br_variant = tunings.br_variant == 2 ? 2 : 0;
    const size_t words = (size_t)count * dp.N;
    uint32_t scale[2];
    (void)make_twiddles(dp.N, scale);
    const int32_t *dtp = scratch_upload(S_NEGA_TP, tp, words, "upload tp");
    const int32_t *dip = scratch_upload(S_NEGA_IP, ip, words, "upload ip");
    uint32_t *dimg = scratch_as<uint32_t>(S_NEGA_IMG, words * 2);
    int32_t *dres = scratch_as<int32_t>(S_NEGA_RES, words);
    launch_bk_transform(stream_, dp, dtp, dimg, key->tw, count, 1, scale);
    launch_negacyclic(stream_, dp, key->tw, dip, dimg, dres, count);
    hip_check(hipGetLastError(), "negacyclic launch");
    d2h(res, dres, words, "download res");
    sync_stream("negacyclic");
}

uint32_t *Engine::upload_pack_image(const DeviceKeyImage *key, const Torus32 *rows, int t, size_t *bytes) {
    ENGINE_DEVICE_SCOPE();
    ensure_init();
    const DevParams &dp = key->dp;
    const size_t words = (size_t)dp.n * t * 2 * dp.N;
    uint32_t scale[2];
    (void)make_twiddles(dp.N, scale);
    uint32_t *img = static_cast<uint32_t *>(recoverable_alloc(words * 2 * 4, "the NTT image of a packing key"));
    int32_t *raw = nullptr;
    try {
        raw = static_cast<int32_t *>(recoverable_alloc(words * 4, "the staging copy of a packing key"));
    } catch (const ApiError &) {
        recoverable_free(img, words * 2 * 4);
        throw;
    }
    hip_check(hipMemcpy(raw, rows, words * 4, hipMemcpyHostToDevice), "upload packing key");
    launch_bk_transform(stream_, dp, raw, img, key->tw, dp.n * t, 2, scale);
    hip_check(hipGetLastError(), "packing key transform launch");
    sync_stream("packing key transform");
    recoverable_free(raw, words * 4);
    *bytes = words * 2 * 4;
    return img;
}

uint32_t *Engine::expand_pack_image(const DeviceKeyImage *key, const uint32_t seed10[10], const Torus32 *body, int t, size_t *bytes) {
    ENGINE_DEVICE_SCOPE();
    ensure_init();
    const DevParams &dp = key->dp;
    const size_t body_words = (size_t)dp.n * t * dp.N, words = body_words * 2;
    uint32_t scale[2];
    (void)make_twiddles(dp.N, scale);
    uint32_t *img = nullptr;
    int32_t *raw = nullptr, *dbody = nullptr;
    try {
        img = static_cast<uint32_t *>(recoverable_alloc(words * 2 * 4, "the NTT image of a packing key"));
        raw = static_cast<int32_t *>(recoverable_alloc(words * 4, "the staging copy of a packing key"));
        dbody = static_cast<int32_t *>(recoverable_alloc(body_words * 4, "the bodies of a compressed packing key"));
    } catch (const ApiError &) {
        recoverable_free(raw, words * 4);
        recoverable_free(img, words * 2 * 4);
        throw;
    }
    h2d_staged(dbody, body, body_words, "upload packing key bodies");
    ExpandBkArgs ea{};
    std::memcpy(ea.seed.key, seed10, sizeof ea.seed.key);
    ea.seed.nonce[0] = seed10[8]; ea.seed.nonce[1] = seed10[9];
    ea.rows = dp.n * t; ea.k = 1; ea.N = dp.N; ea.body = dbody; ea.raw = raw;
    if (!launch_expand_bk(stream_, ea)) fatal("packing key expand: arguments outside what the kernel was built for");
    hip_check(hipGetLastError(), "packing key expand launch");
    launch_bk_transform(stream_, dp, raw, img, key->tw, dp.n * t, 2, scale);
    hip_check(hipGetLastError(), "packing key transform launch");
    sync_stream("packing key expansion");
    recoverable_free(raw, words * 4);
    recoverable_free(dbody, body_words * 4);
    ++seeded_stats.expanded_packing_keys;
    ++seeded_stats.packing_expand_launches;
    *bytes = words * 2 * 4;
    return img;
}

size_t Engine::read_pack_image(const uint32_t *img, size_t bytes, Torus32 *out, size_t capacity) {
    ENGINE_DEVICE_SCOPE();
    const size_t words = bytes / 4;
    if (!out || capacity < words) return words;
    wait_flight();
    hip_check(hipMemcpyAsync(out, img, bytes, hipMemcpyDeviceToHost, stream_), "download packing key image");
    sync_stream("packing key image");
    return words;
}

void Engine::free_pack_image(uint32_t *img, size_t bytes) {
    ENGINE_DEVICE_SCOPE();
    if (!img) return;
    if (inited_) sync_stream("sync before packing key free");
    recoverable_free(img, bytes);
}

void Engine::run_pack(const DeviceKeyImage *key, const uint32_t *img, int t, int basebit, SlotPool *pool, const int32_t *slots,
                      const Torus32 *raw_words, int count, int idx_per_wg, Torus32 *out, bool out_on_device, bool wait) {
    ENGINE_DEVICE_SCOPE();
    const DevParams &dp = key->dp;
    PackArgs a{};
    a.N = dp.N; a.n = dp.n; a.t = t; a.basebit = basebit; a.count = count;
    a.idx_per_wg = idx_per_wg > 0 ? idx_per_wg : 1;
    a.img = img; a.tw = key->tw;
    const size_t out_words = (size_t)2 * dp.N, raw_words_n = (size_t)count * (dp.n + 1);
// ... 237 lines not shown
```

### peba1_amd/csrc/engine.hpp

```cpp
#pragma once
#include <hip/hip_runtime.h>

#include <atomic>
#include <chrono>
#include <cstdint>
#include <string>
#include <vector>

#include "host_keys.hpp"
#include "host_stage.hpp"
#include "br_forms.hpp"
#include "launch_plan.hpp"
#include "kernels.hpp"
#include "pack.hpp"
#include "unpack.hpp"
#include "cmux.hpp"
#include "expand.hpp"
#include "../../include/tfhe_hip.h"

struct DeviceKeyImage {
    tfhe_hip::DevParams dp;
    tfhe_hip::DevKey key;
    bool form_ok[tfhe_hip::BR_FORM_COUNT][3] = {};
    uint32_t *bk_img = nullptr;
    int32_t *ksk = nullptr;
    uint32_t *tw = nullptr;
    size_t bk_img_bytes = 0, ksk_bytes = 0, tw_bytes = 0;
};

namespace tfhe_hip {

void set_error(const std::string &msg);
const std::string &last_error_ref();
[[noreturn]] void fatal(const std::string &msg);
void hip_check(hipError_t e, const char *what);
const char *unsupported_reason(const Params &p);

struct ApiError { std::string msg; };
void set_alloc_cap(long long bytes);
[[noreturn]] void api_fail(const std::string &msg);

constexpr size_t MAX_POOL_SLOTS = (size_t)1 << 29;
constexpr int MAX_PACKED_SAMPLES = 1 << 16;

class SlotPool {
public:
    SlotPool(int ct_words, int ct_stride, size_t capacity);
    ~SlotPool();
    int32_t alloc();
    void retain(int32_t s) { ++ref_[s]; }
    int32_t refs(int32_t s) const { return ref_[s]; }
    void release(int32_t s);
    int32_t *data() { return data_; }
    int ct_stride() const { return stride_; }
    int ct_words() const { return words_; }
    size_t capacity() const { return max_cap_; }
    size_t allocated() const { return cap_; }
    size_t in_use() const { return cap_ - free_.size(); }
    std::vector<int32_t> level;
    std::vector<uint8_t> pending;
    int32_t const_slot[2] = {-1, -1};
private:
    void grow(size_t new_cap);
    int words_, stride_;
    size_t cap_ = 0, max_cap_;
    int32_t *data_ = nullptr;
    std::vector<int32_t> ref_;
    std::vector<int32_t> free_;
};

struct LevelPlan {
    std::vector<RotDesc> rots;
    std::vector<KsDesc> kss;
    std::vector<NotDesc> nots;
    int levels = 0;
    std::vector<int32_t> rot_off, ks_off;
    std::vector<int32_t> not_off;
    std::vector<LinDesc> lins;
    std::vector<int32_t> lin_level_off, lin_launch_off, lin_launch_rank, op_rank;
    int32_t max_rots = 0;
    int32_t max_extracts = 0;
    int nkeys = 1;
    std::vector<int32_t> rot_key;
    std::vector<int32_t> rot_koff, ks_koff;
    std::vector<tfhe_hip::DevKey> dev_keys;
};

class Engine {
public:
    static Engine &get();
    void ensure_init();
    int device() const { return device_; }
    int cu_count() const { return cu_count_; }
    void set_device(int d);
    hipStream_t stream() const { return stream_; }

    DeviceKeyImage *upload_key(const TfheHipCloudKey &ck);
    DeviceKeyImage *upload_compressed_key(const TfheHipCloudKey &ck);
    double last_expand_ms = -1.0;
    void free_key(DeviceKeyImage *img);
    void run_expand_masks(const uint32_t seed10[10], int64_t first_word, int count, uint32_t *out);
    size_t read_key_image(const DeviceKeyImage *img, int which, Torus32 *out, size_t capacity);
    SlotPool *pool_for(const Params &p);
    SlotPool *find_pool(const Params &p) const;

    void write_slot(SlotPool *pool, int32_t slot, const Torus32 *a, Torus32 b);
    void read_slot(SlotPool *pool, int32_t slot, Torus32 *a, Torus32 *b);
    void write_slots_packed(SlotPool *pool, const int32_t *slots, int count, const Torus32 *words, bool words_on_device, bool wait = true);
    void read_slots_packed(SlotPool *pool, const int32_t *slots, int count, Torus32 *words, bool words_on_device, bool wait = true);

    void execute(const std::vector<const DeviceKeyImage *> &keys, SlotPool *pool, LevelPlan &&plan, bool wait = true);
    int last_flush_keys = 0;
    void wait_flight();
    void sync_stream(const char *what);
    void sync_io() { stage_.wait(); }
    void wait_all() { wait_flight(); sync_io(); }
    void wait_event(hipEvent_t ev, const char *what, long long deadline_ms, const std::string &label);
    bool pci_bus_id(char *out, int len);
    long long sync_deadline_ms = 0;
    std::string diag_label;
    bool in_flight() const { return in_flight_; }
    int32_t lut_add(const Torus32 *words, int n_ring);
    void lut_free(int32_t index);
    int32_t spec_add(const ExtractSpec &xs);
    void spec_free(int32_t index);
    void run_raw_rotations(const DeviceKeyImage *key, const Torus32 *lin, int count, const int32_t *lut_index,
                           const Torus32 *polys, int npolys, const int32_t *spec_index, const ExtractSpec *specs, int nspecs,
                           int out_rows, Torus32 *u_out, Torus32 *acc_out, const char *name);
    void run_keyswitch(const DeviceKeyImage *key, const Torus32 *u, int count, Torus32 *out);
    void run_negacyclic(const DeviceKeyImage *key, const int32_t *ip, const Torus32 *tp, Torus32 *res, int count);
    uint32_t *upload_pack_image(const DeviceKeyImage *key, const Torus32 *rows, int t, size_t *bytes);
    uint32_t *expand_pack_image(const DeviceKeyImage *key, const uint32_t seed10[10], const Torus32 *body, int t, size_t *bytes);
    void free_pack_image(uint32_t *img, size_t bytes);
    size_t read_pack_image(const uint32_t *img, size_t bytes, Torus32 *out, size_t capacity);
    void run_pack(const DeviceKeyImage *key, const uint32_t *img, int t, int basebit, SlotPool *pool, const int32_t *slots,
                  const Torus32 *raw_words, int count, int idx_per_wg, Torus32 *out, bool out_on_device, bool wait);

    void run_unpack(const DeviceKeyImage *key, const Torus32 *ring_words, int nring, bool ring_on_device, const int32_t *index,
                    int count, SlotPool *pool, const int32_t *slots, Torus32 *u_out, bool wait, bool seeded = false);

    size_t read_extract_rows(Torus32 *out, size_t capacity);

    void run_lwe_expand(int n, int stride, const Torus32 *record, bool record_on_device, const int32_t *index, int count,
                        SlotPool *pool, const int32_t *slots, Torus32 *rows_out, bool wait);
    size_t read_expand_slots(Torus32 *out, size_t capacity);

    TfheHipStats stats{};
    TfheHipExpandStats expand_stats{};
    TfheHipSeededStats seeded_stats{};
    bool kernel_timing = false;
    LaunchTunings tunings;
    void launch_ks(const DeviceKeyImage *key, const int32_t *u_buf, const KsDesc *descs, int count, int32_t *pool,
                   hipStream_t stream = nullptr, bool presized = false);
    BrPlan plan_br_launch(const DeviceKeyImage *key, int count, bool acc_dump) const;
    struct BrLaunch {
        const int32_t *pool;
        const RotDesc *rots;
        int count;
        int32_t *u_buf;
        int32_t *acc_dbg = nullptr;
        hipStream_t stream = nullptr;
        const DevKey *mk_keys = nullptr;
        const int32_t *mk_rot_keys = nullptr;
        hipEvent_t *mid = nullptr;
        const int32_t *luts = nullptr;
        const ExtractSpec *specs = nullptr;
    };
    void launch_br(const DeviceKeyImage *key, const BrPlan &plan, const BrLaunch &a);
    double run_wg_times(const DeviceKeyImage *key, int width, unsigned long long *wg_times);

private:
    Engine() = default;
    enum Scratch : size_t {
        S_ROTS,
        S_KS,
        S_NOTS,
        S_LINS,
        S_SLOTS,
        S_WORDS,
        S_EXTRACT,
        S_RAW_POOL,
        S_RAW_ACC,
        S_NEGA_TP = S_RAW_POOL, S_NEGA_IP = S_RAW_ACC,
        S_NEGA_IMG,
        S_NEGA_RES,
        S_KS_PARTIAL,
        S_KEYS,
        S_ROT_KEYS,
        S_RAW_LUTS,
        S_RAW_SPECS,
        S_PROBE_POOL, S_PROBE_ROTS, S_PROBE_TIMES, S_PROBE_EXTRACT,
        S_PACK_SLOTS,
        S_PACK_RAW,
        S_PACK_PARTIAL,
        S_PACK_OUT,
        S_UNPACK_RING,
        S_UNPACK_INDEX,
        S_UNPACK_KS,
        S_UNPACK_EXTRACT,
        S_EXPAND_WORDS,
        S_LWE_RECORD,
        S_LWE_INDEX,
        S_LWE_SLOTS,
        S_LWE_ROWS,
        S_SELECT_RING,
        S_SELECT_A,
        S_SELECT_B,
        S_CMUX_D1,
    };
    void *scratch(Scratch idx, size_t bytes);
    template <class T> T *scratch_as(Scratch idx, size_t count, size_t margin = 0) { return static_cast<T *>(scratch(idx, count * sizeof(T) + margin)); }
    template <class T> void h2d(T *dst, const T *src, size_t count, const char *what) {
        hip_check(hipMemcpyAsync(dst, src, count * sizeof(T), hipMemcpyHostToDevice, stream_), what);
    }
    template <class T> void d2h(T *dst, const T *src, size_t count, const char *what) {
        hip_check(hipMemcpyAsync(dst, src, count * sizeof(T), hipMemcpyDeviceToHost, stream_), what);
    }
    template <class T> void h2d_staged(T *dst, const T *src, size_t count, const char *what) {
        T *h = static_cast<T *>(stage_.reserve(count * sizeof(T)));
        std::copy(src, src + count, h);
        h2d(dst, h, count, what);
    }
    template <class T> T *scratch_upload(Scratch idx, const T *src, size_t count, const char *what) {
        T *d = scratch_as<T>(idx, count);
        h2d(d, src, count, what);
        return d;
    }
    struct FlushBuffers { RotDesc *rots; KsDesc *ks; NotDesc *nots; int32_t *u_buf; DevKey *keys; int32_t *rot_keys; LinDesc *lins; };
    FlushBuffers prepare_flush(const std::vector<const DeviceKeyImage *> &keys, LevelPlan &plan);
    void upload_flush(const FlushBuffers &fb, LevelPlan &&plan);
    void run_level(const std::vector<const DeviceKeyImage *> &keys, SlotPool *pool, const FlushBuffers &fb, int L, hipEvent_t &shared_end);
    struct Timed { hipEvent_t e0, e1, e2; bool wide8; int nrot; hipEvent_t em = nullptr; int tail = 0; };
    void finish(bool host_wait, const char *what) { host_wait ? sync_stream(what) : stage_.uploaded(); }
    std::vector<Timed> flight_timed_;
    hipEvent_t flight_base_ = nullptr;
    LevelPlan flight_plan_;
    int flight_levels_ = 0;
    bool in_flight_ = false;
    std::chrono::steady_clock::time_point flight_t0_;
    size_t last_extract_words_ = 0;
    HostStage stage_{*this};
    int device_ = 0;
    int cu_count_ = 256;
    std::atomic<bool> inited_{false};
    hipStream_t stream_ = nullptr;
    unsigned long long *clock_acc_ = nullptr;
    unsigned long long *wg_times_dbg_ = nullptr;
    size_t timing_used_ = 0;
    hipEvent_t next_timing_event();
    std::vector<hipEvent_t> timing_events_;
    std::vector<int32_t> spec_nout_;
    std::vector<SlotPool *> pools_;
    std::vector<void *> scratch_ptr_;
    std::vector<size_t> scratch_size_;
    size_t last_expand_words_ = 0;
public:
    TfheHipSeededLweStats seeded_lwe_stats{};

    struct SelectorImage { uint32_t *img = nullptr, *tw = nullptr; size_t img_bytes = 0, tw_bytes = 0; };
    SelectorImage *upload_selector(const Params &p, const Torus32 *words, int nbits);
    void free_selector(SelectorImage *sel);
    void run_select(const SelectorImage *sel, const Params &p, int nbits, const Torus32 *ring, int M, bool ring_on_device,
                    Torus32 *out, bool out_on_device);
    void run_cmux(const SelectorImage *sel, const Params &p, int bit, const Torus32 *d1, const Torus32 *d0, int count, Torus32 *out);
    double last_select_ms();
private:
    hipEvent_t select_e0_ = nullptr, select_e1_ = nullptr;
    bool select_timed_ = false;
};

}
```

### peba1_amd/csrc/launch_plan.hpp

```cpp
#pragma once
#include <algorithm>
#include <climits>
#include <cstddef>
#include <cstdint>

#include "br_forms.hpp"

namespace tfhe_hip {

struct LaunchTunings {
    int br_variant = -1;
    int br8_max_rotations = 1 << 30;
    int br_tail8 = 1;
    int br_digit_table = 1;
    int ks_target_blocks = 32768;
    int ks_max_splits = 48;
    int ks_split_ties = 0;
    int ks_tile = 16;
    int ks_index = 1;
};

inline void fill_form_ok(bool form_ok[BR_FORM_COUNT][3], int N, int l, int Bgbit) {
    for (int f = 0; f < BR_FORM_COUNT; ++f)
        for (int t = 0; t < 3; ++t) form_ok[f][t] = br_form_admissible(f, N, l, Bgbit, t);
}

struct BrPlan { int form; int tables; int tail; };

inline BrPlan plan_br(const bool form_ok[BR_FORM_COUNT][3], int N, int l, const LaunchTunings &t, int cu_count, int count,
                      bool stamps, bool acc_dump) {
    int form;
    if (t.br_variant == 4 && N == 1024) form = BR_FORM_WAVE2;
    else if (t.br_variant == 2 || N == 2048) form = BR_FORM_SPLIT;
    else if (t.br8_max_rotations > 0 && count <= std::min(t.br8_max_rotations, cu_count) && l >= 2 && !stamps)
        form = BR_FORM_WAVE8;
    else form = BR_FORM_WIDE4;
    if (stamps && N == 1024) form = BR_FORM_WIDE4;
    int tables = t.br_digit_table < 0 || t.br_digit_table > 2 ? 0 : t.br_digit_table;
    if (!form_ok[form][tables]) {
        static const int order[BR_FORM_COUNT] = {BR_FORM_WIDE4, BR_FORM_SPLIT, BR_FORM_WAVE2, BR_FORM_WAVE8};
        int pick_f = -1, pick_t = 0;
        for (int k = -1; k < BR_FORM_COUNT && pick_f < 0; ++k) {
            const int f = k < 0 ? form : order[k];
            if (f == BR_FORM_WAVE8 && count > cu_count) continue;
            for (int tt : {tables, 2, 0})
                if (form_ok[f][tt]) { pick_f = f; pick_t = tt; break; }
        }
        if (pick_f < 0) return BrPlan{-1, 0, 0};
        form = pick_f; tables = pick_t;
    }
    const int round = 2 * cu_count, tail = count % round;
    const bool split = form == BR_FORM_WIDE4 && t.br_tail8 && count > round && tail > 0 &&
                       tail <= std::min(t.br8_max_rotations, cu_count) && l >= 2 && !acc_dump && !stamps &&
                       form_ok[BR_FORM_WAVE8][tables];
    return BrPlan{form, tables, split ? tail : 0};
}

constexpr int KS_CHUNK = 8192;
struct KsShape { int nin, ks_t, ks_basebit, ct_stride; };

inline int ks_threads(const KsShape &p) { return ((p.ct_stride / 4 + 63) / 64) * 64; }

enum KsForm { KS_FORM_PERGATE = 0, KS_FORM_STRIP = 1, KS_FORM_INDEX = 2 };
struct KsPlan { int form; int tile; };

inline int ks_tile_size(const LaunchTunings &t) { return (t.ks_tile > 16 && !t.ks_index) ? 16 : t.ks_tile; }

inline KsPlan plan_ks(const LaunchTunings &t, int count, const KsShape &p) {
    const int tile = ks_tile_size(t), threads = ks_threads(p);
    const bool tiled = (tile == 16 || tile == 24 || tile == 32) && count >= 2 * tile && p.ks_t == 8 && p.ks_basebit == 2 &&
                       t.ks_max_splits > 1 && (p.nin + t.ks_max_splits - 1) / t.ks_max_splits <= 64 &&
                       (threads == 128 || threads == 192 || threads == 320);
    if (!tiled) return KsPlan{KS_FORM_PERGATE, 0};
    return KsPlan{t.ks_index ? KS_FORM_INDEX : KS_FORM_STRIP, tile};
}

inline bool ks_tiled(const LaunchTunings &t, int count, const KsShape &p) { return plan_ks(t, count, p).form != KS_FORM_PERGATE; }

inline int ks_splits(const LaunchTunings &t, int cu_count, int cnt, const KsShape &p) {
    int splits = 1;
    const KsPlan plan = plan_ks(t, cnt, p);
    if (plan.form != KS_FORM_PERGATE) {
        const int tile = plan.tile;
        const int threads = ks_threads(p);
        int per_cu = std::max(1, (tile == 16 ? 16 : tile == 24 ? 12 : 8) / (threads / 64));
        if (plan.form == KS_FORM_STRIP) {
            const size_t lds = (size_t)16 * threads * 16 + (size_t)tile * 65 * 4;
            per_cu = std::max(1, std::min((int)((160 * 1024) / lds), 8 / (threads / 64)));
        }
        const long long slots = (long long)cu_count * per_cu;
        const long long tiles = (cnt + tile - 1) / tile;
        const int lo = std::max(2, (p.nin + 63) / 64);
        double best = -1.0;
        for (int sp = lo; sp <= t.ks_max_splits; ++sp) {
            const long long blocks = tiles * sp, rounds = (blocks + slots - 1) / slots;
            const double eff = (double)blocks / (double)(rounds * slots);
            if (t.ks_split_ties ? eff >= best - 1e-9 : eff > best + 1e-9) { best = eff; splits = sp; }
        }
    } else {
        while (splits < t.ks_max_splits && cnt * splits * 2 <= t.ks_target_blocks) splits *= 2;
    }
    return splits;
}

struct LevelCost {
    const int32_t *width = nullptr;
    const double *us = nullptr;
    int n = 0;
    int period = 0;
};

inline long long level_cost_fold(const LevelCost &c, long long width) {
    const long long top = c.width[c.n - 1];
    if (width <= top || c.period <= 0 || c.period > top - c.width[0]) return 0;
    return (width - top + c.period - 1) / c.period;
}

inline double level_cost_at(const LevelCost &c, long long width) {
    if (width <= 0 || c.n <= 0) return 0.0;
    if (width <= c.width[0] || c.n == 1) return c.us[0];
    const long long top = c.width[c.n - 1], fold = level_cost_fold(c, width);
    if (fold > 0) return level_cost_at(c, width - fold * c.period) + (double)fold * (c.us[c.n - 1] - level_cost_at(c, top - c.period));
    const int32_t *hi = std::lower_bound(c.width, c.width + c.n, (int32_t)std::min<long long>(width, top));
    const int j = (int)(hi - c.width);
    return c.us[j - 1] + (c.us[j] - c.us[j - 1]) * (double)(width - c.width[j - 1]) / (double)(c.width[j] - c.width[j - 1]);
}

inline int level_cost_steps(const LevelCost &c, long long width, int dir, long long *out, int most) {
    if (c.n <= 0) return 0;
    const long long shift = level_cost_fold(c, width) * c.period, at = width - shift;
    int count = 0;
    if (dir < 0) {
        for (int j = (int)(std::lower_bound(c.width, c.width + c.n, (int32_t)std::min<long long>(at, INT32_MAX)) - c.width) - 1;
             j >= 0 && count < most; --j)
            out[count++] = c.width[j] + shift;
    } else {
        for (int j = (int)(std::upper_bound(c.width, c.width + c.n, (int32_t)std::min<long long>(at, INT32_MAX)) - c.width);
             j < c.n && count < most; ++j)
            out[count++] = c.width[j] + shift;
    }
    return count;
}

struct LevelCostEntry {
    int n, N, k, l, Bgbit, ks_t, ks_basebit;
    int cus;
    int br_variant, br8_max_rotations, br_tail8, br_digit_table, ks_tile, ks_index, ks_max_splits, ks_target_blocks,
        ks_split_ties;
    int count;
    const int32_t *width;
    const double *us;
};
#if __has_include("level_cost_tables.inc")
#include "level_cost_tables.inc"
#else
#warning "level_cost_tables.inc is missing (run tools/level_cost_inc.py before peba1_amd/csrc/build.sh): this library knows no level-cost table and the tuning level_slack does nothing"
static constexpr LevelCostEntry LEVEL_COST_TABLES[1] = {};
static constexpr int LEVEL_COST_TABLE_COUNT = 0;
#endif

struct LevelCostSet { int n, N, k, l, Bgbit, ks_t, ks_basebit; };

inline LevelCost level_cost_table(const LevelCostSet &p, int cus, const LaunchTunings &t) {
    for (int i = 0; i < LEVEL_COST_TABLE_COUNT; ++i) {
        const LevelCostEntry &e = LEVEL_COST_TABLES[i];
        if (e.n == p.n && e.N == p.N && e.k == p.k && e.l == p.l && e.Bgbit == p.Bgbit && e.ks_t == p.ks_t &&
            e.ks_basebit == p.ks_basebit && e.cus == cus && e.br_variant == t.br_variant &&
            e.br8_max_rotations == t.br8_max_rotations && e.br_tail8 == t.br_tail8 && e.br_digit_table == t.br_digit_table &&
            e.ks_tile == t.ks_tile && e.ks_index == t.ks_index && e.ks_max_splits == t.ks_max_splits &&
            e.ks_target_blocks == t.ks_target_blocks && e.ks_split_ties == t.ks_split_ties)
            return LevelCost{e.width, e.us, e.count, 2 * e.cus};
    }
    return LevelCost{};
}

inline double level_cost_us(int width, const LevelCostSet &p, int cus, const LaunchTunings &t) {
    const LevelCost c = level_cost_table(p, cus, t);
    return c.n ? level_cost_at(c, width) : -1.0;
}

inline size_t ks_partial_bytes(const LaunchTunings &t, int cu_count, int count, const KsShape &p) {
    size_t most = 0;
    const int chunk = ks_tiled(t, count, p) ? KS_CHUNK : count;
    for (int done = 0; done < count; done += chunk) {
        const int cnt = std::min(chunk, count - done), splits = ks_splits(t, cu_count, cnt, p);
        if (splits > 1) most = std::max(most, (size_t)cnt * splits * p.ct_stride * 4);
    }
    return most;
}

}
```

### peba1_amd/csrc/shim.cpp

```cpp
#include <cstddef>
#include <cstdio>
#include <cstdlib>
#include <cstring>
#include <algorithm>
#include <string>
#include <vector>

#include "scheduler.hpp"
#include "shim_internal.hpp"

using namespace tfhe_hip;

namespace {

constexpr uint32_t ARRAY_MAGIC = 0x7F4E11A5u;

constexpr int MIRROR_PREFIX_WORDS = 4;
constexpr uint64_t MIRROR_MARKER = 0x7F4E5A3D1E5AA11Cull;

void record_gate2(int code, LweSample *result, const LweSample *ca, const LweSample *cb,
                  const TFheGateBootstrappingCloudKeySet *bk) {
    guarded([&] {
        auto g = recorder_lock();
        record_gate2_locked(code, result, ca, cb, bk);
// ... 650 lines not shown

TfheHipLutMulti *tfhe_hip_new_lut_multi_from_tables(const TFheGateBootstrappingParameterSet *params, Torus32 step, int32_t slots,
                                                    int32_t nout, const int32_t *levels) {
    const char *who = "tfhe_hip_new_lut_multi_from_tables";
    if (!params || !params->tgsw_params || !params->tgsw_params->tlwe_params) { set_error(std::string(who) + ": null parameter set"); return nullptr; }
    const int32_t N = params->tgsw_params->tlwe_params->N;
    if (N < 1 || N > LUT_STRIDE) { set_error(std::string(who) + ": ring size out of range"); return nullptr; }
    if (!levels) { set_error(std::string(who) + ": null levels"); return nullptr; }
    if (step & 1) { set_error(std::string(who) + ": step must be even (the test polynomial is the constant step/2)"); return nullptr; }
    if (slots < 2 || N % slots != 0) { set_error(std::string(who) + ": slots must be at least 2 and divide N = " + std::to_string(N)); return nullptr; }
    if (nout < 1 || nout > XS_MAX_OUT) { set_error(std::string(who) + ": nout must be 1..4"); return nullptr; }
    ExtractSpec xs{};
    xs.nout = nout;
    const uint32_t half = (uint32_t)(step / 2);
    for (int m = 0; m < nout; ++m) {
        const int32_t *L = levels + (size_t)m * slots;
        int nt = 0;
        for (int j = 1; j < slots; ++j) {
            const int64_t w = (int64_t)L[slots - 1 - j] - (int64_t)L[slots - j];
            if (w == 0) continue;
            if (w > XS_MAX_WEIGHT || w < -XS_MAX_WEIGHT) { set_error(std::string(who) + ": neighbouring levels differ by more than 8"); return nullptr; }
            if (nt == XS_MAX_TAPS) { set_error(std::string(who) + ": an output would need more than 8 taps"); return nullptr; }
            xs.index[m][nt] = j * (N / slots);
            xs.weight[m][nt] = (int32_t)w;
            ++nt;
        }
        if (nt == 0) { set_error(std::string(who) + ": an output with equal levels in every sector needs no tap (it is a constant)"); return nullptr; }
        xs.ntaps[m] = nt;
        xs.out_c0[m] = (int32_t)(half * ((uint32_t)L[0] + (uint32_t)L[slots - 1]));
    }
    const std::vector<Torus32> words((size_t)N, (Torus32)half);
    return make_lut_multi(who, N, words.data(), xs);
}

void tfhe_hip_delete_lut_multi(TfheHipLutMulti *mo) {
    if (!mo) return;
    if (mo->magic != LUTM_MAGIC) { set_error("tfhe_hip_delete_lut_multi: not a multi-output LUT (or already deleted)"); return; }
    auto g = recorder_lock();
    if (mo->lut.dev >= 0 || mo->dev_spec >= 0) {
        guarded([&] { forget_lutm_locked(mo->lut.dev, mo->dev_spec); });
        if (mo->lut.dev >= 0) Engine::get().lut_free(mo->lut.dev);
        if (mo->dev_spec >= 0) Engine::get().spec_free(mo->dev_spec);
    }
    mo->magic = 0;
    mo->lut.magic = 0;
    delete mo;
}

int32_t tfhe_hip_lut_multi_nout(const TfheHipLutMulti *mo) {
    if (!mo || mo->magic != LUTM_MAGIC) { set_error("tfhe_hip_lut_multi_nout: null or deleted multi-output LUT"); return -1; }
    return mo->spec.nout;
}

int32_t tfhe_hip_lut_multi_output(const TfheHipLutMulti *mo, int32_t m, int32_t *tap_index, int32_t *tap_weight, Torus32 *out_c0) {
    if (!mo || mo->magic != LUTM_MAGIC) { set_error("tfhe_hip_lut_multi_output: null or deleted multi-output LUT"); return -1; }
    if (m < 0 || m >= mo->spec.nout) { set_error("tfhe_hip_lut_multi_output: no such output"); return -1; }
    for (int t = 0; t < mo->spec.ntaps[m]; ++t) {
        if (tap_index) tap_index[t] = mo->spec.index[m][t];
        if (tap_weight) tap_weight[t] = mo->spec.weight[m][t];
    }
    if (out_c0) *out_c0 = mo->spec.out_c0[m];
    return mo->spec.ntaps[m];
}

const Torus32 *tfhe_hip_lut_multi_words(const TfheHipLutMulti *mo, int32_t *count) {
    if (!mo || mo->magic != LUTM_MAGIC) { set_error("tfhe_hip_lut_multi_words: null or deleted multi-output LUT"); if (count) *count = 0; return nullptr; }
    if (count) *count = mo->lut.N;
    return mo->lut.words.data();
}

void tfhe_hip_lut_bootstrap_multi(const TfheHipLutMulti *mo, LweSample *const *result, int32_t nin, const LweSample *const *in,
                                  const int32_t *coef, Torus32 c0, const TFheGateBootstrappingCloudKeySet *bk) {
    guarded([&] {
        auto g = recorder_lock();
        lutm_check_results(mo, result);
        lutm_entry(mo, nin, in, coef, bk);
        record_lutm_locked(mo->lut.dev, mo->dev_spec, mo->spec.nout, result, nin, in, coef, c0, bk);
    });
}

int tfhe_hip_lut_bootstrap_multi_batch(const TfheHipLutMulti *mo, LweSample *const *result, int32_t nin,
                                       const LweSample *const *in, const int32_t *coef, Torus32 c0, int32_t count,
                                       const TFheGateBootstrappingCloudKeySet *bk) {
    return record_batch([&] {
        lutm_check_results(mo, result);
        lutm_entry(mo, nin, in, coef, bk);
        for (int32_t i = 0; i < count; ++i) {
            const LweSample *ops[3] = {&in[0][i], nin > 1 ? &in[1][i] : nullptr, nin > 2 ? &in[2][i] : nullptr};
            LweSample *res[XS_MAX_OUT] = {nullptr, nullptr, nullptr, nullptr};
            for (int m = 0; m < mo->spec.nout; ++m) res[m] = result[m] ? &result[m][i] : nullptr;
            record_lutm_locked(mo->lut.dev, mo->dev_spec, mo->spec.nout, res, nin, ops, coef, c0, bk);
        }
    });
}

static void linear_args_check(const char *who, const void *result, int32_t nin, const void *in, const int32_t *coef,
                              const TFheGateBootstrappingCloudKeySet *bk) {
    if (nin < 1 || nin > TFHE_HIP_LINEAR_MAX_IN) api_fail(std::string(who) + ": nin must be 1..16");
    if (!result) api_fail(std::string(who) + ": null result");
    if (!in || !coef) api_fail(std::string(who) + ": null operand or coefficient list");
    for (int32_t i = 0; i < nin; ++i)
        if (!static_cast<const void *const *>(in)[i]) api_fail(std::string(who) + ": null operand");
    if (!bk || !bk->bk) api_fail("null cloud key");
}
static void linear_sample_check(const LweSample *s, const TFheGateBootstrappingCloudKeySet *bk) {
    if (header_of(s)->n != bk->bk->p.n) api_fail("ciphertext used with a key of different LWE dimension than the one it was allocated for");
}

void tfhe_hip_linear(LweSample *result, int32_t nin, const LweSample *const *in, const int32_t *coef, Torus32 c0,
                     const TFheGateBootstrappingCloudKeySet *bk) {
    static_assert(TFHE_HIP_LINEAR_MAX_IN == LIN_MAX_IN && LIN_MAX_IN == LIN_DESC_MAX_IN, "one limit, from the header to the kernel");
    guarded([&] {
        linear_args_check("tfhe_hip_linear", result, nin, in, coef, bk);
        linear_sample_check(result, bk);
        for (int32_t i = 0; i < nin; ++i) linear_sample_check(in[i], bk);
        auto g = recorder_lock();
        record_linear_locked(result, nin, in, coef, c0, bk);
    });
}

int tfhe_hip_linear_batch(LweSample *result, int32_t nin, const LweSample *const *in, const int32_t *coef, Torus32 c0,
                          int32_t count, const TFheGateBootstrappingCloudKeySet *bk) {
    auto g = recorder_lock();
    const int rc = record_batch([&] {
        linear_args_check("tfhe_hip_linear_batch", result, nin, in, coef, bk);
        if (count > 0) {
            linear_sample_check(result, bk);
            for (int32_t k = 0; k < nin; ++k) linear_sample_check(in[k], bk);
        }
        for (int32_t i = 0; i < count; ++i) {
            const LweSample *ops[LIN_MAX_IN];
            for (int32_t k = 0; k < nin; ++k) ops[k] = &in[k][i];
            record_linear_locked(&result[i], nin, ops, coef, c0, bk);
        }
    });
    if (rc == 0 && !deferred_mode())
        return guarded_rc([&] { for (int32_t i = 0; i < count; ++i) sync_sample_locked(&result[i]); return 0; });
    return rc;
}

int tfhe_hip_set_tuning(const char *name, int64_t value) {
    auto g = recorder_lock();
    if (name && std::strcmp(name, "ks_tile") == 0) {
        if (value != 0 && value != 16 && value != 24 && value != 32) { set_error("ks_tile must be 0, 16, 24 or 32"); return -1; }
        Engine::get().tunings.ks_tile = (int)value;
        return 0;
    }
    if (name && std::strcmp(name, "ks_index") == 0) { Engine::get().tunings.ks_index = value != 0; return 0; }
    if (name && std::strcmp(name, "ks_max_splits") == 0) {
        if (value < 1 || value > 64) { set_error("ks_max_splits must be in [1, 64]"); return -1; }
        Engine::get().tunings.ks_max_splits = (int)value;
        return 0;
    }
    if (name && std::strcmp(name, "br_digit_table") == 0) { Engine::get().tunings.br_digit_table = (int)value; return 0; }
    if (name && std::strcmp(name, "br8_max_rotations") == 0) { Engine::get().tunings.br8_max_rotations = (int)value; return 0; }
    if (name && std::strcmp(name, "br_tail8") == 0) { Engine::get().tunings.br_tail8 = (int)value; return 0; }
    if (name && std::strcmp(name, "br_variant") == 0) { Engine::get().tunings.br_variant = (int)value; return 0; }
    if (name && set_recorder_tuning_locked(name, value != 0)) return 0;
    if (name && std::strcmp(name, "sync_deadline_ms") == 0) { Engine::get().sync_deadline_ms = value > 0 ? (long long)value : 0; return 0; }
    set_error(std::string("tfhe_hip_set_tuning: unknown name ") + (name ? name : "(null)"));
    return -1;
}

void tfhe_hip_get_stats(TfheHipStats *out) {
    auto g = recorder_lock();
    Engine::get().wait_flight();
    if (out) *out = Engine::get().stats;
}
void tfhe_hip_reset_stats(void) {
    auto g = recorder_lock();
    Engine::get().stats = TfheHipStats{};
    Engine::get().expand_stats = TfheHipExpandStats{};
    Engine::get().seeded_stats = TfheHipSeededStats{};
    Engine::get().seeded_lwe_stats = TfheHipSeededLweStats{};
}
void tfhe_hip_get_seeded_stats(TfheHipSeededStats *out) {
    auto g = recorder_lock();
    if (out) *out = Engine::get().seeded_stats;
}
void tfhe_hip_get_expand_stats(TfheHipExpandStats *out) {
    auto g = recorder_lock();
    if (out) *out = Engine::get().expand_stats;
}
void tfhe_hip_set_kernel_timing(int on) { Engine::get().kernel_timing = on != 0; }
int tfhe_hip_last_flush_keys(void) {
    auto g = recorder_lock();
    return Engine::get().last_flush_keys;
}
int tfhe_hip_set_batch_keys(int on) {
    auto g = recorder_lock();
    return set_batch_keys_locked(on != 0) ? 1 : 0;
}

}

#include "pack_host.cpp"
#include "unpack_host.cpp"
#include "select_host.cpp"
#include "compressed_host.cpp"
#include "seeded_host.cpp"
#include "seeded_lwe_host.cpp"
#include "test_entries.cpp"
#include "recorder.cpp"
```

### peba1_amd/kernel_id.py

```python
import hashlib
import os

CSRC = os.path.join(os.path.dirname(os.path.abspath(__file__)), "csrc")
KERNEL_FILES = ("kernels.hip", "kernels.hpp", "ntt_wave.hpp", "ntt_field.hpp", "br_forms.hpp", "ks_index_asm.inc", "br8_body.inc",
                "build.sh")


def kernels_sha16():
    h = hashlib.sha256()
    for name in KERNEL_FILES:
        with open(os.path.join(CSRC, name), "rb") as f:
            data = f.read()
        h.update(name.encode() + b"\0" + str(len(data)).encode() + b"\0")
        h.update(data)
    return h.hexdigest()[:16]
```

### peba1_amd/lib.py

```python
import ctypes as C
import os

_HERE = os.path.dirname(os.path.abspath(__file__))
LIB_PATH = os.environ.get("PEBA1_TFHE_HIP_LIB") or os.path.join(_HERE, "libtfhe-hip.so")
CIRCUITS_PATH = os.path.join(_HERE, "libpeba1-circuits.so")


class LweSample(C.Structure):
    _fields_ = [("a", C.POINTER(C.c_int32)), ("b", C.c_int32), ("slot", C.c_int32),
                ("current_variance", C.c_double)]


class LweParams(C.Structure):
    _fields_ = [("n", C.c_int32), ("alpha_min", C.c_double), ("alpha_max", C.c_double)]


class TLweParams(C.Structure):
    _fields_ = [("N", C.c_int32), ("k", C.c_int32), ("alpha_min", C.c_double), ("alpha_max", C.c_double)]


class TGswParams(C.Structure):
    _fields_ = [("l", C.c_int32), ("Bgbit", C.c_int32), ("Bg", C.c_int32), ("halfBg", C.c_int32),
                ("maskMod", C.c_uint32), ("tlwe_params", C.POINTER(TLweParams)), ("kpl", C.c_int32),
                ("offset", C.c_uint32)]


class ParameterSet(C.Structure):
    _fields_ = [("ks_t", C.c_int32), ("ks_basebit", C.c_int32), ("in_out_params", C.POINTER(LweParams)),
                ("tgsw_params", C.POINTER(TGswParams))]


class CloudKeySet(C.Structure):
    _fields_ = [("params", C.POINTER(ParameterSet)), ("bk", C.c_void_p), ("bkFFT", C.c_void_p)]


class SecretKeySet(C.Structure):
    _fields_ = [("params", C.POINTER(ParameterSet)), ("lwe_key", C.c_void_p), ("tgsw_key", C.c_void_p),
                ("cloud", CloudKeySet)]


class Stats(C.Structure):
    _fields_ = [("blind_rotates", C.c_uint64), ("keyswitches", C.c_uint64), ("linear_ops", C.c_uint64),
                ("levels", C.c_uint64), ("flushes", C.c_uint64), ("br_launches", C.c_uint64),
                ("ms_blind_rotate", C.c_double), ("ms_keyswitch", C.c_double), ("ms_flush_wall", C.c_double),
                ("ms_blind_rotate_busy", C.c_double), ("reused_gates", C.c_uint64),
                ("br8_launches", C.c_uint64), ("br8_rotations", C.c_uint64), ("ms_blind_rotate8", C.c_double),
                ("clk_shader_cycles", C.c_uint64), ("clk_ref_ticks", C.c_uint64), ("dead_gates", C.c_uint64),
                ("folded_gates", C.c_uint64),
                ("br_wide4_launches", C.c_uint64), ("br_split_launches", C.c_uint64),
                ("br_wave8_launches", C.c_uint64), ("br_wave2_launches", C.c_uint64),
                ("br_tables0_launches", C.c_uint64), ("br_tables1_launches", C.c_uint64),
                ("br_tables2_launches", C.c_uint64), ("lut_rotations", C.c_uint64),
                ("multi_rotations", C.c_uint64), ("multi_outputs", C.c_uint64)]


class StatsAll(Stats):
    _fields_ = [("lincomb_ops", C.c_uint64), ("lincomb_launches", C.c_uint64),
                ("ks_pergate_launches", C.c_uint64), ("ks_strip_launches", C.c_uint64), ("ks_index_launches", C.c_uint64)]


class StatsWhole(StatsAll):
    _fields_ = [("unpacked_samples", C.c_uint64), ("unpack_launches", C.c_uint64)]


class ExpandStats(C.Structure):
    _fields_ = [("expanded_keys", C.c_uint64), ("expand_launches", C.c_uint64)]


class SeededStats(C.Structure):
    _fields_ = [("expanded_packing_keys", C.c_uint64), ("packing_expand_launches", C.c_uint64),
                ("seeded_unpacked_samples", C.c_uint64), ("seeded_unpack_launches", C.c_uint64)]


class SeededLweStats(C.Structure):
    _fields_ = [("seeded_imported_samples", C.c_uint64), ("seeded_import_launches", C.c_uint64)]


STATS_FIELDS = [f for f, _ in Stats._fields_] + [f for f, _ in StatsAll._fields_]
UNPACK_STATS_FIELDS = [f for f, _ in StatsWhole._fields_]
EXPAND_STATS_FIELDS = [f for f, _ in ExpandStats._fields_]
SEEDED_STATS_FIELDS = [f for f, _ in SeededStats._fields_]
SEEDED_LWE_STATS_FIELDS = [f for f, _ in SeededLweStats._fields_]


PS = C.POINTER(ParameterSet)
CK = C.POINTER(CloudKeySet)
SK = C.POINTER(SecretKeySet)
LS = C.POINTER(LweSample)
I32P = C.POINTER(C.c_int32)
U32P = C.POINTER(C.c_uint32)

_GATE2 = ["bootsAND", "bootsOR", "bootsXOR", "bootsXNOR", "bootsNAND", "bootsNOR", "bootsANDNY", "bootsANDYN",
          "bootsORNY", "bootsORYN"]
SIGNATURES = {
    "new_gate_bootstrapping_ciphertext_array": (LS, [C.c_int32, PS]),
    "delete_gate_bootstrapping_ciphertext_array": (None, [C.c_int32, LS]),
    "new_gate_bootstrapping_ciphertext": (LS, [PS]),
    "delete_gate_bootstrapping_ciphertext": (None, [LS]),
    "bootsCONSTANT": (None, [LS, C.c_int32, CK]),
    "bootsNOT": (None, [LS, LS, CK]),
    "bootsCOPY": (None, [LS, LS, CK]),
    "bootsMUX": (None, [LS, LS, LS, LS, CK]),
    "new_default_gate_bootstrapping_parameters": (PS, [C.c_int32]),
    "new_random_gate_bootstrapping_secret_keyset": (SK, [PS]),
    "delete_gate_bootstrapping_parameters": (None, [PS]),
    "delete_gate_bootstrapping_secret_keyset": (None, [SK]),
    "delete_gate_bootstrapping_cloud_keyset": (None, [CK]),
    "bootsSymEncrypt": (None, [LS, C.c_int32, SK]),
    "bootsSymDecrypt": (C.c_int32, [LS, SK]),
    "modSwitchFromTorus32": (C.c_int32, [C.c_int32, C.c_int32]),
    "modSwitchToTorus32": (C.c_int32, [C.c_int32, C.c_int32]),
    "export_tfheGateBootstrappingParameterSet_toFile": (None, [C.c_void_p, PS]),
    "new_tfheGateBootstrappingParameterSet_fromFile": (PS, [C.c_void_p]),
    "export_tfheGateBootstrappingCloudKeySet_toFile": (None, [C.c_void_p, CK]),
    "new_tfheGateBootstrappingCloudKeySet_fromFile": (CK, [C.c_void_p]),
    "export_tfheGateBootstrappingSecretKeySet_toFile": (None, [C.c_void_p, SK]),
    "new_tfheGateBootstrappingSecretKeySet_fromFile": (SK, [C.c_void_p]),
    "export_gate_bootstrapping_ciphertext_toFile": (None, [C.c_void_p, LS, PS]),
    "import_gate_bootstrapping_ciphertext_fromFile": (None, [C.c_void_p, LS, PS]),
    "tfhe_hip_test_wg_times": (C.c_int, [CK, C.c_int32, C.POINTER(C.c_uint64), C.POINTER(C.c_double)]),
    "tfhe_hip_last_error": (C.c_char_p, []),
    "tfhe_hip_clear_error": (None, []),
    "tfhe_hip_set_device": (C.c_int, [C.c_int]),
    "tfhe_hip_get_device": (C.c_int, []),
    "tfhe_hip_device_pci_bus_id": (C.c_int, [C.c_char_p, C.c_int]),
    "tfhe_hip_new_parameters": (PS, [C.c_int32] * 7 + [C.c_double] * 3),
    "tfhe_hip_new_p2048_parameters": (PS, []),
    "tfhe_hip_new_secret_keyset_seeded": (SK, [PS, C.c_uint64]),
    "tfhe_hip_new_secret_keyset_seeded_host": (SK, [PS, C.c_uint64]),
    "tfhe_hip_set_encrypt_seed": (None, [C.c_uint64]),
    "tfhe_hip_randomness_is_seeded": (C.c_int, []),
    "tfhe_hip_test_chacha20_block": (None, [C.POINTER(C.c_uint32), C.c_uint64, C.POINTER(C.c_uint32), C.POINTER(C.c_uint32)]),
    "tfhe_hip_key_lwe": (I32P, [SK, C.POINTER(C.c_int64)]),
    "tfhe_hip_key_tlwe": (I32P, [SK, C.POINTER(C.c_int64)]),
    "tfhe_hip_key_bk": (I32P, [CK, C.POINTER(C.c_int64)]),
    "tfhe_hip_key_ksk": (I32P, [CK, C.POINTER(C.c_int64)]),
    "tfhe_hip_sample_words": (C.c_int32, [PS]),
    "tfhe_hip_export_samples": (C.c_int, [LS, C.c_int32, PS, I32P]),
    "tfhe_hip_import_samples": (C.c_int, [LS, C.c_int32, PS, I32P]),
    "tfhe_hip_export_samples_device": (C.c_int, [LS, C.c_int32, PS, C.c_void_p]),
    "tfhe_hip_import_samples_device": (C.c_int, [LS, C.c_int32, PS, C.c_void_p]),
    "tfhe_hip_export_samples_device_async": (C.c_int, [LS, C.c_int32, PS, C.c_void_p]),
    "tfhe_hip_import_samples_device_async": (C.c_int, [LS, C.c_int32, PS, C.c_void_p]),
    "tfhe_hip_stream": (C.c_void_p, []),
    "tfhe_hip_sync_samples": (C.c_int, [LS, C.c_int32]),
    "tfhe_hip_set_deferred": (None, [C.c_int]),
    "tfhe_hip_get_deferred": (C.c_int, []),
    "tfhe_hip_flush": (C.c_int, []),
    "tfhe_hip_flush_async": (C.c_int, []),
    "tfhe_hip_wait": (C.c_int, []),
    "tfhe_hip_stream_sync": (C.c_int, []),
    "tfhe_hip_wait_event": (C.c_int, [C.c_void_p, C.c_char_p]),
    "tfhe_hip_set_diag_label": (None, [C.c_char_p]),
    "tfhe_hip_gate_batch": (C.c_int, [C.c_int, LS, LS, LS, C.c_int32, CK]),
    "tfhe_hip_gate3": (None, [C.c_int, C.c_int, LS, LS, LS, LS, CK]),
    "tfhe_hip_gate3_batch": (C.c_int, [C.c_int, C.c_int, LS, LS, LS, LS, C.c_int32, CK]),
    "tfhe_hip_new_lut": (C.c_void_p, [PS, I32P]),
    "tfhe_hip_new_lut_constant": (C.c_void_p, [PS, C.c_int32]),
    "tfhe_hip_new_lut_from_table": (C.c_void_p, [PS, I32P, C.c_int32]),
    "tfhe_hip_delete_lut": (None, [C.c_void_p]),
    "tfhe_hip_lut_words": (I32P, [C.c_void_p, I32P]),
    "tfhe_hip_lut_bootstrap": (None, [C.c_void_p, LS, C.c_int32, C.POINTER(LS), I32P, C.c_int32, CK]),
    "tfhe_hip_lut_bootstrap_batch": (C.c_int, [C.c_void_p, LS, C.c_int32, C.POINTER(LS), I32P, C.c_int32, C.c_int32, CK]),
    "tfhe_hip_new_lut_multi": (C.c_void_p, [C.c_void_p, C.c_int32, I32P, I32P, I32P, I32P]),
    "tfhe_hip_new_lut_multi_from_tables": (C.c_void_p, [PS, C.c_int32, C.c_int32, C.c_int32, I32P]),
    "tfhe_hip_delete_lut_multi": (None, [C.c_void_p]),
    "tfhe_hip_lut_multi_nout": (C.c_int32, [C.c_void_p]),
    "tfhe_hip_lut_multi_output": (C.c_int32, [C.c_void_p, C.c_int32, I32P, I32P, I32P]),
    "tfhe_hip_lut_multi_words": (I32P, [C.c_void_p, I32P]),
    "tfhe_hip_lut_bootstrap_multi": (None, [C.c_void_p, C.POINTER(LS), C.c_int32, C.POINTER(LS), I32P, C.c_int32, CK]),
    "tfhe_hip_lut_bootstrap_multi_batch": (C.c_int, [C.c_void_p, C.POINTER(LS), C.c_int32, C.POINTER(LS), I32P, C.c_int32,
                                                     C.c_int32, CK]),
    "tfhe_hip_linear": (None, [LS, C.c_int32, C.POINTER(LS), I32P, C.c_int32, CK]),
    "tfhe_hip_linear_batch": (C.c_int, [LS, C.c_int32, C.POINTER(LS), I32P, C.c_int32, C.c_int32, CK]),
    "tfhe_hip_sym_encrypt_torus": (None, [LS, C.c_int32, SK]),
    "tfhe_hip_sym_phase": (C.c_int32, [LS, SK]),
    "tfhe_hip_set_tuning": (C.c_int, [C.c_char_p, C.c_int64]),
    "tfhe_hip_test_form_admissible": (C.c_int, [C.c_int, C.c_int32, C.c_int32, C.c_int32, C.c_int]),
    "tfhe_hip_test_set_alloc_cap": (None, [C.c_int64]),
    "tfhe_hip_test_stage_place": (C.c_int, [C.c_int64, C.c_int64, C.c_int32, C.c_int64, C.POINTER(C.c_int64)]),
    "tfhe_hip_get_stats": (None, [C.POINTER(StatsWhole)]),
    "tfhe_hip_reset_stats": (None, []),
    "tfhe_hip_set_kernel_timing": (None, [C.c_int]),
    "tfhe_hip_last_flush_keys": (C.c_int, []),
    "tfhe_hip_set_batch_keys": (C.c_int, [C.c_int]),
    "tfhe_hip_test_schedule": (C.c_int, [I32P, C.c_int32, C.c_int32, C.c_int32, I32P]),
    "tfhe_hip_test_level_plan": (C.c_int, [I32P, I32P, C.c_int32, C.c_int32, C.c_int32, C.c_int32] + [I32P] * 9),
    "tfhe_hip_test_level_plan3": (C.c_int, [I32P, I32P, C.c_int32, C.c_int32, C.c_int32, C.c_int32] + [I32P] * 9),
    "tfhe_hip_test_level_plan_lut": (C.c_int, [I32P, I32P, C.c_int32, C.c_int32, C.c_int32, C.c_int32, C.c_int32] + [I32P] * 10),
    "tfhe_hip_test_level_plan_multi": (C.c_int, [I32P, I32P, C.c_int32, C.c_int32, C.c_int32, C.c_int32, C.c_int32, I32P,
                                                 C.c_int32] + [I32P] * 10),
    "tfhe_hip_test_level_plan_lin": (C.c_int, [I32P, I32P, C.c_int32, C.c_int32, C.c_int32, C.c_int32, C.c_int32, I32P,
                                               C.c_int32, I32P, C.c_int32] + [I32P] * 16),
    "tfhe_hip_test_level_plan_full": (C.c_int, [I32P, I32P, C.c_int32, C.c_int32, C.c_int32, C.c_int32, C.c_int32, I32P,
                                                C.c_int32, I32P, C.c_int32] + [I32P] * 18),
    "tfhe_hip_test_level_slack": (C.c_int, [I32P, C.c_int32, C.c_int32, C.c_int32, I32P, C.POINTER(C.c_double), C.c_int32, C.c_int32, I32P,
                                            I32P, C.POINTER(C.c_double)]),
    "tfhe_hip_test_level_cost": (C.c_int, [C.c_int32] * 9 + [C.POINTER(C.c_double)]),
    "tfhe_hip_test_set_level_cost": (C.c_int, [I32P, C.POINTER(C.c_double), C.c_int32]),
    "tfhe_hip_last_level_slack": (C.c_int, [C.POINTER(C.c_double)]),
    "tfhe_hip_test_br_plan": (C.c_int, [C.c_int32] * 3 + [I32P, C.c_int32, C.c_int32, C.c_int32, I32P]),
    "tfhe_hip_test_ks_plan": (C.c_int, [C.c_int32] * 5 + [I32P, C.c_int32, C.c_int32, C.POINTER(C.c_int64)]),
    "tfhe_hip_test_ks_plan_form": (C.c_int, [C.c_int32] * 5 + [I32P, C.c_int32, C.c_int32, C.POINTER(C.c_int64)]),
    "tfhe_hip_kernel_negacyclic":(C.c_int, [CK, I32P, I32P, I32P, C.c_int32]),
    "tfhe_hip_kernel_bootstrap_woks": (C.c_int, [CK, I32P, C.c_int32, I32P, I32P]),
    "tfhe_hip_kernel_lut_bootstrap_woks": (C.c_int, [CK, I32P, C.c_int32, I32P, I32P, C.c_int32, I32P, I32P]),
    "tfhe_hip_kernel_lut_bootstrap_multi_woks": (C.c_int, [CK, I32P, C.c_int32, I32P, I32P, C.c_int32, I32P, I32P, C.c_int32,
                                                           I32P, I32P]),
    "tfhe_hip_kernel_keyswitch": (C.c_int, [CK, I32P, C.c_int32, I32P]),
    "tfhe_hip_new_packing_key": (C.c_void_p, [SK, C.c_int32, C.c_int32]),
    "tfhe_hip_new_packing_key_seeded": (C.c_void_p, [SK, C.c_int32, C.c_int32, C.c_uint64]),
    "tfhe_hip_new_packing_key_from_words": (C.c_void_p, [PS, C.c_int32, C.c_int32, I32P]),
    "tfhe_hip_delete_packing_key": (None, [C.c_void_p]),
    "tfhe_hip_packing_key_words": (I32P, [C.c_void_p, C.POINTER(C.c_int64)]),
    "tfhe_hip_packing_key_decomposition": (C.c_int, [C.c_void_p, I32P, I32P]),
    "tfhe_hip_pack_samples": (C.c_int, [C.c_void_p, LS, C.c_int32, CK, I32P]),
    "tfhe_hip_pack_samples_device": (C.c_int, [C.c_void_p, LS, C.c_int32, CK, C.c_void_p]),
    "tfhe_hip_packed_phase": (C.c_int, [SK, I32P, I32P]),
    "tfhe_hip_packed_decrypt_bits": (C.c_int, [SK, I32P, C.c_int32, I32P]),
    "tfhe_hip_test_pack_bounds": (C.c_int, [C.c_int32, C.c_int32, C.c_int32]),
    "tfhe_hip_kernel_pack": (C.c_int, [C.c_void_p, CK, I32P, C.c_int32, C.c_int32, I32P]),
    "tfhe_hip_ring_encrypt": (C.c_int, [SK, I32P, I32P]),
    "tfhe_hip_ring_encrypt_seeded": (C.c_int, [SK, I32P, I32P, C.c_uint64]),
    "tfhe_hip_ring_encrypt_bits": (C.c_int, [SK, I32P, C.c_int32, I32P]),
    "tfhe_hip_ring_encrypt_bits_seeded": (C.c_int, [SK, I32P, C.c_int32, I32P, C.c_uint64]),
    "tfhe_hip_unpack_samples": (C.c_int, [CK, I32P, C.c_int32, I32P, C.c_int32, LS]),
    "tfhe_hip_unpack_samples_scattered": (C.c_int, [CK, I32P, C.c_int32, I32P, C.c_int32, C.POINTER(LS)]),
    "tfhe_hip_unpack_samples_device": (C.c_int, [CK, C.c_void_p, C.c_int32, I32P, C.c_int32, LS]),
    "tfhe_hip_kernel_ring_extract": (C.c_int, [CK, I32P, C.c_int32, I32P, C.c_int32, I32P]),
    "tfhe_hip_new_compressed_cloud_key": (C.c_void_p, [SK]),
    "tfhe_hip_new_compressed_cloud_key_seeded": (C.c_void_p, [SK, C.c_uint64, U32P]),
    "tfhe_hip_new_compressed_cloud_key_from_words": (C.c_void_p, [PS, U32P, I32P, I32P]),
    "tfhe_hip_delete_compressed_cloud_key": (None, [C.c_void_p]),
    "tfhe_hip_compressed_key_seed": (U32P, [C.c_void_p]),
    "tfhe_hip_compressed_key_bk_body": (I32P, [C.c_void_p, C.POINTER(C.c_int64)]),
    "tfhe_hip_compressed_key_ksk_body": (I32P, [C.c_void_p, C.POINTER(C.c_int64)]),
    "tfhe_hip_compressed_key_bytes": (C.c_int64, [C.c_void_p]),
    "tfhe_hip_expand_cloud_key_host": (CK, [C.c_void_p]),
    "tfhe_hip_expand_cloud_key": (CK, [C.c_void_p]),
    "tfhe_hip_export_compressed_cloud_key_toFile": (None, [C.c_void_p, C.c_void_p]),
    "tfhe_hip_new_compressed_cloud_key_fromFile": (C.c_void_p, [C.c_void_p]),
    "tfhe_hip_kernel_expand_masks": (C.c_int, [U32P, C.c_int64, C.c_int32, U32P]),
    "tfhe_hip_test_key_image": (C.c_int64, [CK, C.c_int, I32P, C.c_int64]),
    "tfhe_hip_last_expand_ms": (C.c_double, []),
    "tfhe_hip_get_expand_stats": (None, [C.POINTER(ExpandStats)]),
    "tfhe_hip_get_seeded_stats": (None, [C.POINTER(SeededStats)]),
    "tfhe_hip_new_compressed_packing_key": (C.c_void_p, [SK, C.c_int32, C.c_int32]),
    "tfhe_hip_new_compressed_packing_key_seeded": (C.c_void_p, [SK, C.c_int32, C.c_int32, C.c_uint64, U32P]),
    "tfhe_hip_new_compressed_packing_key_from_words": (C.c_void_p, [PS, C.c_int32, C.c_int32, U32P, I32P]),
    "tfhe_hip_delete_compressed_packing_key": (None, [C.c_void_p]),
    "tfhe_hip_compressed_packing_key_seed": (U32P, [C.c_void_p]),
    "tfhe_hip_compressed_packing_key_body": (I32P, [C.c_void_p, C.POINTER(C.c_int64)]),
    "tfhe_hip_compressed_packing_key_decomposition": (C.c_int, [C.c_void_p, I32P, I32P]),
    "tfhe_hip_compressed_packing_key_bytes": (C.c_int64, [C.c_void_p]),
    "tfhe_hip_expand_packing_key_host": (C.c_void_p, [C.c_void_p]),
    "tfhe_hip_expand_packing_key": (C.c_void_p, [C.c_void_p]),
    "tfhe_hip_export_compressed_packing_key_toFile": (None, [C.c_void_p, C.c_void_p]),
    "tfhe_hip_new_compressed_packing_key_fromFile": (C.c_void_p, [C.c_void_p]),
    "tfhe_hip_ring_encrypt_compressed": (C.c_int, [SK, I32P, I32P]),
    "tfhe_hip_ring_encrypt_compressed_seeded": (C.c_int, [SK, I32P, I32P, U32P, C.c_uint64]),
    "tfhe_hip_ring_encrypt_bits_compressed": (C.c_int, [SK, I32P, C.c_int32, I32P]),
    "tfhe_hip_ring_encrypt_bits_compressed_seeded": (C.c_int, [SK, I32P, C.c_int32, I32P, U32P, C.c_uint64]),
    "tfhe_hip_ring_expand_host": (C.c_int, [I32P, C.c_int32, I32P]),
    "tfhe_hip_unpack_samples_seeded": (C.c_int, [CK, I32P, C.c_int32, I32P, C.c_int32, LS]),
    "tfhe_hip_unpack_samples_seeded_scattered": (C.c_int, [CK, I32P, C.c_int32, I32P, C.c_int32, C.POINTER(LS)]),
    "tfhe_hip_unpack_samples_seeded_device": (C.c_int, [CK, C.c_void_p, C.c_int32, I32P, C.c_int32, LS]),
    "tfhe_hip_kernel_ring_extract_seeded": (C.c_int, [CK, I32P, C.c_int32, I32P, C.c_int32, I32P]),
    "tfhe_hip_test_pack_image": (C.c_int64, [C.c_void_p, CK, I32P, C.c_int64]),
    "tfhe_hip_test_extract_rows": (C.c_int64, [I32P, C.c_int64]),
    "tfhe_hip_sym_encrypt_bits_compressed": (C.c_int, [SK, I32P, C.c_int32, I32P]),
    "tfhe_hip_sym_encrypt_bits_compressed_seeded": (C.c_int, [SK, I32P, C.c_int32, I32P, U32P, C.c_uint64]),
    "tfhe_hip_sym_encrypt_torus_compressed": (C.c_int, [SK, I32P, C.c_int32, I32P]),
    "tfhe_hip_sym_encrypt_torus_compressed_seeded": (C.c_int, [SK, I32P, C.c_int32, I32P, U32P, C.c_uint64]),
    "tfhe_hip_lwe_expand_host": (C.c_int, [I32P, C.c_int32, C.c_int32, I32P, C.c_int32, I32P]),
    "tfhe_hip_import_samples_seeded": (C.c_int, [PS, I32P, C.c_int32, I32P, C.c_int32, LS]),
    "tfhe_hip_import_samples_seeded_scattered": (C.c_int, [PS, I32P, C.c_int32, I32P, C.c_int32, C.POINTER(LS)]),
    "tfhe_hip_import_samples_seeded_device": (C.c_int, [PS, C.c_void_p, C.c_int32, I32P, C.c_int32, LS]),
    "tfhe_hip_kernel_lwe_expand": (C.c_int, [PS, I32P, C.c_int32, I32P, C.c_int32, I32P]),
    "tfhe_hip_test_expand_slots": (C.c_int64, [I32P, C.c_int64]),
    "tfhe_hip_get_seeded_lwe_stats": (None, [C.POINTER(SeededLweStats)]),
    "tfhe_hip_tgsw_words": (C.c_int64, [PS]),
    "tfhe_hip_tgsw_encrypt_bits": (C.c_int, [SK, I32P, C.c_int32, I32P]),
    "tfhe_hip_tgsw_encrypt_bits_seeded": (C.c_int, [SK, I32P, C.c_int32, I32P, C.c_uint64]),
    "tfhe_hip_new_selector": (C.c_void_p, [PS, I32P, C.c_int32]),
    "tfhe_hip_delete_selector": (None, [C.c_void_p]),
    "tfhe_hip_selector_bits": (C.c_int32, [C.c_void_p]),
    "tfhe_hip_ring_select": (C.c_int, [C.c_void_p, I32P, C.c_int32, I32P]),
    "tfhe_hip_ring_select_device": (C.c_int, [C.c_void_p, C.c_void_p, C.c_int32, C.c_void_p]),
    "tfhe_hip_last_select_ms": (C.c_double, []),
    "tfhe_hip_kernel_ring_cmux": (C.c_int, [C.c_void_p, C.c_int32, I32P, I32P, C.c_int32, I32P]),
    "tfhe_hip_test_select_bounds": (C.c_int, [C.c_int32, C.c_int32, C.c_int32]),
}
for _g in _GATE2:
    SIGNATURES[_g] = (None, [LS, LS, LS, CK])
_lib = None


def load():
    global _lib
    if _lib is None:
        if not os.path.exists(LIB_PATH):
            raise RuntimeError(
                f"{LIB_PATH} is missing: build it with `python -c 'import __graft_entry__ as g; g.build()'` "
                "(peba1_amd has no CPU fallback)")
        L = C.CDLL(LIB_PATH, mode=C.RTLD_GLOBAL)
        for name, (res, args) in SIGNATURES.items():
            f = getattr(L, name)
            f.restype = res
            f.argtypes = args
        _lib = L
    return _lib
```

Measured before the change: 110,000.

## Add MFMA int8 byte-plane matrix key switch for wide levels

Adds a key-switch form that converts the key-switching key once into signed byte planes and computes the key switch as int8 matrix products on MFMA units (32x32x32 i8), recombining the four byte planes into 32-bit results. The planner picks this form when the tiled path applies and the level width reaches ks_matrix_min (default 512). It replaces the scalar gather-and-add key switch with dense matrix work, aiming to cut the key-switch share of each level. The cost is an extra device-memory image of the key, a one-time conversion kernel, and a chance that the matrix path loses at narrow widths.

```diff
diff --git a/include/tfhe_hip.h b/include/tfhe_hip.h
--- a/include/tfhe_hip.h
+++ b/include/tfhe_hip.h
@@ -156,6 +156,10 @@
     uint64_t expand_launches;
 } TfheHipExpandStats;
 void tfhe_hip_get_expand_stats(TfheHipExpandStats *out);
+typedef struct TfheHipKsMatrixStats {
+    uint64_t ks_matrix_launches;
+} TfheHipKsMatrixStats;
+void tfhe_hip_get_ks_matrix_stats(TfheHipKsMatrixStats *out);
 typedef struct TfheHipSeededStats {
     uint64_t expanded_packing_keys;
     uint64_t packing_expand_launches;
@@ -219,6 +223,9 @@
                           int32_t cu_count, int32_t count, int64_t *out6);
 int tfhe_hip_test_ks_plan_form(int32_t n, int32_t N, int32_t k, int32_t ks_t, int32_t ks_basebit, const int32_t *tunings5,
                                int32_t cu_count, int32_t count, int64_t *out7);
+int tfhe_hip_test_ks_plan_form2(int32_t n, int32_t N, int32_t k, int32_t ks_t, int32_t ks_basebit, const int32_t *tunings7,
+                                int32_t has_image, int32_t cu_count, int32_t count, int64_t *out7);
+int tfhe_hip_test_ks_byte_planes(const uint32_t *words, int32_t count, int8_t *planes4);
 int tfhe_hip_test_wg_times(const TFheGateBootstrappingCloudKeySet *bk, int32_t width, uint64_t *times4, double *launch_ms);
 
 typedef struct TfheHipPackingKey TfheHipPackingKey;
@@ -363,6 +370,8 @@
                                              Torus32 *acc_out);
 int tfhe_hip_kernel_keyswitch(const TFheGateBootstrappingCloudKeySet *bk, const Torus32 *u,
                               int32_t count, Torus32 *out);
+int tfhe_hip_kernel_keyswitch_matrix(const TFheGateBootstrappingCloudKeySet *bk, const Torus32 *u,
+                                     int32_t count, Torus32 *out);
 int tfhe_hip_kernel_pack(const TfheHipPackingKey *key, const TFheGateBootstrappingCloudKeySet *bk, const Torus32 *sample_words,
                          int32_t count, int32_t idx_per_wg, Torus32 *out_words);
 int tfhe_hip_kernel_ring_extract(const TFheGateBootstrappingCloudKeySet *bk, const Torus32 *ring_words, int32_t nring,
diff --git a/peba1_amd/api.py b/peba1_amd/api.py
--- a/peba1_amd/api.py
+++ b/peba1_amd/api.py
@@ -262,6 +262,12 @@
     return out
 
 
+def ks_matrix_stats():
+    s = _l.KsMatrixStats()
+    _l.load().tfhe_hip_get_ks_matrix_stats(C.byref(s))
+    return {"ks_matrix_launches": s.ks_matrix_launches}
+
+
 def expand_stats():
     s = _l.ExpandStats()
     _l.load().tfhe_hip_get_expand_stats(C.byref(s))
@@ -1145,3 +1151,13 @@
     if rc != 0:
         raise RuntimeError(last_error())
     return out
+
+
+def kernel_keyswitch_matrix(key, u):
+    p = key.params
+    u = np.ascontiguousarray(u, dtype=np.int32).reshape(-1, p.k * p.N + 1)
+    out = np.zeros((u.shape[0], p.words), dtype=np.int32)
+    rc = _l.load().tfhe_hip_kernel_keyswitch_matrix(key.cloud, _i32p(u), u.shape[0], _i32p(out))
+    if rc != 0:
+        raise RuntimeError(last_error())
+    return out
diff --git a/peba1_amd/csrc/engine.cpp b/peba1_amd/csrc/engine.cpp
--- a/peba1_amd/csrc/engine.cpp
+++ b/peba1_amd/csrc/engine.cpp
@@ -508,7 +508,29 @@
     recoverable_free(img->bk_img, img->bk_img_bytes);
     recoverable_free(img->ksk, img->ksk_bytes);
     recoverable_free(img->tw, img->tw_bytes);
+    recoverable_free(img->ks_planes, img->ks_planes_bytes);
     delete img;
+}
+
+static_assert(KS_MATRIX_SPAN == KSM_WAVES * KSM_CHUNK && KS_MATRIX_TILE == KSM_GATES, "launch_plan.hpp plans what ks_matrix.hip runs");
+bool Engine::ensure_ks_planes(const DeviceKeyImage *key) {
+    ENGINE_DEVICE_SCOPE();
+    if (key->ks_planes) return true;
+    const DevParams &dp = key->dp;
+    if (!ks_matrix_shape_ok(dp.k * dp.N, dp.ks_t, dp.ks_basebit)) return false;
+    const size_t bytes = ks_matrix_image_bytes(dp.k * dp.N, dp.ct_stride);
+    uint8_t *img = nullptr;
+    try {
+        img = static_cast<uint8_t *>(recoverable_alloc(bytes, "the byte-plane image of a key-switching key"));
+    } catch (const ApiError &) {
+        return false;
+    }
+    if (!launch_ksk_planes(stream_, dp, key->key, img)) { recoverable_free(img, bytes); return false; }
+    hip_check(hipGetLastError(), "ksk_planes launch");
+    sync_stream("ksk_planes");
+    key->ks_planes = img;
+    key->ks_planes_bytes = bytes;
+    return true;
 }
 
 static std::vector<int32_t> pad_rows(const int32_t *src, size_t rows, size_t words, size_t stride) {
@@ -704,11 +726,18 @@
     if (!stream) stream = stream_;
     const DevParams &dp = key->dp;
     const KsShape shape = ks_shape(dp);
-    const size_t bytes = ks_partial_bytes(tunings, cu_count_, count, shape);
+    const bool matrix = presized && key->ks_planes != nullptr;
+    const size_t bytes = ks_partial_bytes(tunings, cu_count_, count, shape, matrix);
     if (presized && bytes > (scratch_size_.size() > S_KS_PARTIAL ? scratch_size_[S_KS_PARTIAL] : 0))
         fatal("launch_ks: the key-switch partial sums were not sized by execute()");
     int32_t *partial = bytes ? static_cast<int32_t *>(scratch(S_KS_PARTIAL, bytes)) : nullptr;
-    const KsPlan plan = plan_ks(tunings, count, shape);
+    const KsPlan plan = plan_ks(tunings, count, shape, matrix);
+    if (plan.form == KS_FORM_MATRIX) {
+        ++ks_matrix_stats.ks_matrix_launches;
+        if (!launch_keyswitch_matrix(stream, dp, key->ks_planes, u_buf, descs, count, pool))
+            fatal("launch_ks: the planned matrix key switch has no kernel for this shape");
+        return;
+    }
     const int chunk = plan.form != KS_FORM_PERGATE ? KS_CHUNK : count;
     for (int done = 0; done < count; done += chunk) {
         const int cnt = std::min(chunk, count - done), splits = ks_splits(tunings, cu_count_, cnt, shape);
@@ -749,8 +778,12 @@
     fb.u_buf = scratch_as<int32_t>(S_EXTRACT, (size_t)(std::max(plan.max_rots, plan.max_extracts) + 1) * key->dp.u_stride);
     size_t partial = 0;
     const std::vector<int32_t> &ks_shares = nkeys == 1 ? plan.ks_off : plan.ks_koff;
-    for (size_t sg = 0; sg + 1 < ks_shares.size(); ++sg)
-        partial = std::max(partial, ks_partial_bytes(tunings, cu_count_, ks_shares[sg + 1] - ks_shares[sg], ks_shape(key->dp)));
+    for (size_t sg = 0; sg + 1 < ks_shares.size(); ++sg) {
+        const DeviceKeyImage *share_key = keys[nkeys == 1 ? 0 : sg % (size_t)nkeys];
+        const int width = ks_shares[sg + 1] - ks_shares[sg];
+        const bool matrix = plan_ks(tunings, width, ks_shape(key->dp), true).form == KS_FORM_MATRIX && ensure_ks_planes(share_key);
+        partial = std::max(partial, ks_partial_bytes(tunings, cu_count_, width, ks_shape(key->dp), matrix));
+    }
     if (partial) (void)scratch(S_KS_PARTIAL, partial);
     if (nkeys > 1) {
         fb.keys = scratch_as<DevKey>(S_KEYS, (size_t)nkeys);
@@ -1016,6 +1049,29 @@
     std::vector<int32_t> res((size_t)count * dp.ct_stride);
     d2h(res.data(), dpool, res.size(), "download ks");
     sync_stream("keyswitch");
+    unpad_rows(out, res.data(), (size_t)count, (size_t)dp.n + 1, (size_t)dp.ct_stride);
+    stats.keyswitches += (uint64_t)count;
+}
+
+void Engine::run_keyswitch_matrix(const DeviceKeyImage *key, const Torus32 *u, int count, Torus32 *out) {
+    ENGINE_DEVICE_SCOPE();
+    wait_flight();
+    const DevParams &dp = key->dp;
+    if (count <= 0) api_fail("keyswitch_matrix: no rows");
+    if (!ks_matrix_shape_ok(dp.k * dp.N, dp.ks_t, dp.ks_basebit)) api_fail("keyswitch_matrix: the key's shape has no matrix form");
+    const std::vector<int32_t> padded = pad_rows(u, (size_t)count, (size_t)dp.k * dp.N + 1, (size_t)dp.u_stride);
+    const int32_t *u_buf = scratch_upload(S_EXTRACT, padded.data(), padded.size(), "upload u");
+    std::vector<KsDesc> ks(count);
+    for (int c = 0; c < count; ++c) ks[c] = KsDesc{c, -1, 0, c};
+    const KsDesc *dks = scratch_upload(S_KS, ks.data(), ks.size(), "upload ks");
+    int32_t *dpool = scratch_as<int32_t>(S_RAW_POOL, (size_t)count * dp.ct_stride);
+    if (!ensure_ks_planes(key)) api_fail("keyswitch_matrix: out of device memory for the byte-plane image of the key");
+    ++ks_matrix_stats.ks_matrix_launches;
+    if (!launch_keyswitch_matrix(stream_, dp, key->ks_planes, u_buf, dks, count, dpool)) fatal("keyswitch_matrix: no kernel for this shape");
+    hip_check(hipGetLastError(), "keyswitch_matrix launch");
+    std::vector<int32_t> res((size_t)count * dp.ct_stride);
+    d2h(res.data(), dpool, res.size(), "download ks");
+    sync_stream("keyswitch_matrix");
     unpad_rows(out, res.data(), (size_t)count, (size_t)dp.n + 1, (size_t)dp.ct_stride);
     stats.keyswitches += (uint64_t)count;
 }
diff --git a/peba1_amd/csrc/engine.hpp b/peba1_amd/csrc/engine.hpp
--- a/peba1_amd/csrc/engine.hpp
+++ b/peba1_amd/csrc/engine.hpp
@@ -16,6 +16,7 @@
 #include "unpack.hpp"
 #include "cmux.hpp"
 #include "expand.hpp"
+#include "ks_matrix.hpp"
 #include "../../include/tfhe_hip.h"
 
 struct DeviceKeyImage {
@@ -26,6 +27,8 @@
     int32_t *ksk = nullptr;
     uint32_t *tw = nullptr;
     size_t bk_img_bytes = 0, ksk_bytes = 0, tw_bytes = 0;
+    mutable uint8_t *ks_planes = nullptr;
+    mutable size_t ks_planes_bytes = 0;
 };
 
 namespace tfhe_hip {
@@ -128,6 +131,8 @@
                            const Torus32 *polys, int npolys, const int32_t *spec_index, const ExtractSpec *specs, int nspecs,
                            int out_rows, Torus32 *u_out, Torus32 *acc_out, const char *name);
     void run_keyswitch(const DeviceKeyImage *key, const Torus32 *u, int count, Torus32 *out);
+    void run_keyswitch_matrix(const DeviceKeyImage *key, const Torus32 *u, int count, Torus32 *out);
+    bool ensure_ks_planes(const DeviceKeyImage *key);
     void run_negacyclic(const DeviceKeyImage *key, const int32_t *ip, const Torus32 *tp, Torus32 *res, int count);
     uint32_t *upload_pack_image(const DeviceKeyImage *key, const Torus32 *rows, int t, size_t *bytes);
     uint32_t *expand_pack_image(const DeviceKeyImage *key, const uint32_t seed10[10], const Torus32 *body, int t, size_t *bytes);
@@ -147,6 +152,7 @@
 
     TfheHipStats stats{};
     TfheHipExpandStats expand_stats{};
+    TfheHipKsMatrixStats ks_matrix_stats{};
     TfheHipSeededStats seeded_stats{};
     bool kernel_timing = false;
     LaunchTunings tunings;
diff --git a/peba1_amd/csrc/ks_matrix.hip b/peba1_amd/csrc/ks_matrix.hip
--- /dev/null
+++ b/peba1_amd/csrc/ks_matrix.hip
@@ -0,0 +1,176 @@
+#include "ks_matrix.hpp"
+
+namespace tfhe_hip {
+
+typedef int ksm_v4 __attribute__((ext_vector_type(4)));
+typedef int ksm_v16 __attribute__((ext_vector_type(16)));
+
+__global__ __launch_bounds__(256) void ksk_planes_kernel(DevParams p, DevKey key, uint4 *__restrict__ image, long long total) {
+    const long long id = (long long)blockIdx.x * 256 + threadIdx.x;
+    if (id >= total) return;
+    const int lane = (int)(id & 63), plane = (int)((id >> 6) & 3);
+    const long long ti = id >> 8;
+    const int nin = p.k * p.N;
+    const int i = (int)(ti % nin), wt = (int)(ti / nin);
+    const int w = wt * KSM_WORDS + (lane & 31), h = lane >> 5;
+    uint32_t out[4] = {0u, 0u, 0u, 0u};
+    if (w < p.ct_stride) {
+#pragma unroll
+        for (int r = 0; r < 4; ++r) {
+            const size_t row = ((size_t)i * 8 + (size_t)(4 * h + r)) * 3;
+#pragma unroll
+            for (int v = 1; v < 4; ++v) {
+                int8_t s[4];
+                ks_byte_planes((uint32_t)key.ksk[(row + (size_t)(v - 1)) * p.ct_stride + w], s);
+                out[r] |= (uint32_t)(uint8_t)s[plane] << (8 * v);
+            }
+        }
+    }
+    image[id] = make_uint4(out[0], out[1], out[2], out[3]);
+}
+
+__global__ __launch_bounds__(KSM_WAVES * 64) void keyswitch_matrix_kernel(DevParams p, const uint4 *__restrict__ image,
+                                                                          const int32_t *__restrict__ u_buf,
+                                                                          const KsDesc *__restrict__ descs, int count,
+                                                                          int32_t *__restrict__ pool, int tiles, int wtiles, int per) {
+    constexpr int MS = KSM_GATES / 32;
+    constexpr int REPS = KSM_GATES / 8;
+    constexpr int BLOCK = KSM_CHUNK * KSM_GATES;
+    static_assert(BLOCK == 16 * MS * 64 && KSM_CHUNK == 32 && (16 * MS) % KSM_WAVES == 0, "one LDS block serves both uses");
+    __shared__ uint32_t lds[KSM_WAVES * BLOCK];
+    const int bid = (int)blockIdx.x, vid = (bid & 7) * per + (bid >> 3);
+    if (vid >= tiles * wtiles) return;
+    const int wt = vid / tiles, g0 = (vid - wt * tiles) * KSM_GATES;
+    const int tid = (int)threadIdx.x, wave = tid >> 6, lane = tid & 63;
+    const int nin = p.k * p.N, span = nin / KSM_WAVES, i_lo = wave * span, i_hi = i_lo + span;
+    uint32_t *su = lds + wave * BLOCK;
+    const int part = lane & 7, h = lane >> 5;
+
+    int src0[REPS], src1[REPS];
+    uint32_t keep0[REPS], keep1[REPS];
+    const KsDesc dfirst = descs[g0];
+#pragma unroll
+    for (int rep = 0; rep < REPS; ++rep) {
+        const int g = g0 + rep * 8 + (lane >> 3);
+        const KsDesc d = descs[g < count ? g : g0];
+        keep0[rep] = g < count ? ~0u : 0u;
+        keep1[rep] = g < count && d.u1 >= 0 ? ~0u : 0u;
+        src0[rep] = g < count ? d.u0 : dfirst.u0;
+        src1[rep] = keep1[rep] ? d.u1 : src0[rep];
+    }
+
+    ksm_v16 acc[MS][4];
+#pragma unroll
+    for (int ms = 0; ms < MS; ++ms)
+#pragma unroll
+        for (int pl = 0; pl < 4; ++pl)
+#pragma unroll
+            for (int r = 0; r < 16; ++r) acc[ms][pl][r] = 0;
+
+    const uint4 *bsrc = image + (size_t)wt * (size_t)nin * 256 + lane;
+    uint4 b[4][4];
+#pragma unroll
+    for (int s = 0; s < 3; ++s)
+#pragma unroll
+        for (int pl = 0; pl < 4; ++pl) b[s][pl] = bsrc[(size_t)(i_lo + s) * 256 + pl * 64];
+
+    for (int ic = i_lo; ic < i_hi; ic += KSM_CHUNK) {
+#pragma unroll
+        for (int rep = 0; rep < REPS; ++rep) {
+            uint4 v = *reinterpret_cast<const uint4 *>(u_buf + (size_t)src0[rep] * p.u_stride + ic + 4 * part);
+            const uint4 v1 = *reinterpret_cast<const uint4 *>(u_buf + (size_t)src1[rep] * p.u_stride + ic + 4 * part);
+            const uint32_t off = p.ks_prec_offset;
+            v.x = ((v.x + off) & keep0[rep]) + (v1.x & keep1[rep]); v.y = ((v.y + off) & keep0[rep]) + (v1.y & keep1[rep]);
+            v.z = ((v.z + off) & keep0[rep]) + (v1.z & keep1[rep]); v.w = ((v.w + off) & keep0[rep]) + (v1.w & keep1[rep]);
+            const int col = (rep * 8 + (lane >> 3)) ^ (part << 3);
+            su[(4 * part + 0) * KSM_GATES + col] = v.x;
+            su[(4 * part + 1) * KSM_GATES + col] = v.y;
+            su[(4 * part + 2) * KSM_GATES + col] = v.z;
+            su[(4 * part + 3) * KSM_GATES + col] = v.w;
+        }
+        __builtin_amdgcn_fence(__ATOMIC_RELEASE, "wavefront");
+        __builtin_amdgcn_wave_barrier();
+        __builtin_amdgcn_fence(__ATOMIC_ACQUIRE, "wavefront");
+        for (int ii = 0; ii < KSM_CHUNK; ii += 4) {
+#pragma unroll
+            for (int s = 0; s < 4; ++s) {
+                const int i = ic + ii + s, inext = i + 3 < i_hi ? i + 3 : i_hi - 1;
+#pragma unroll
+                for (int pl = 0; pl < 4; ++pl) b[(s + 3) & 3][pl] = bsrc[(size_t)inext * 256 + pl * 64];
+                ksm_v4 a[MS];
+#pragma unroll
+                for (int ms = 0; ms < MS; ++ms) {
+                    const uint32_t x = su[(ii + s) * KSM_GATES + ((ms * 32 + (lane & 31)) ^ ((((ii + s) >> 2) & 7) << 3))];
+                    const uint32_t y = x >> (24 - 8 * h);
+#pragma unroll
+                    for (int r = 0; r < 4; ++r) a[ms][r] = (int)(1u << (((y >> (6 - 2 * r)) & 3u) << 3));
+                }
+#pragma unroll
+                for (int ms = 0; ms < MS; ++ms)
+#pragma unroll
+                    for (int pl = 0; pl < 4; ++pl) {
+                        const uint4 bw = b[s][pl];
+                        const ksm_v4 bv = {(int)bw.x, (int)bw.y, (int)bw.z, (int)bw.w};
+                        acc[ms][pl] = __builtin_amdgcn_mfma_i32_32x32x32_i8(a[ms], bv, acc[ms][pl], 0, 0, 0);
+                    }
+                __builtin_amdgcn_sched_barrier(0);
+            }
+        }
+        __builtin_amdgcn_fence(__ATOMIC_RELEASE, "wavefront");
+        __builtin_amdgcn_wave_barrier();
+    }
+
+    uint32_t o[16 * MS];
+#pragma unroll
+    for (int ms = 0; ms < MS; ++ms)
+#pragma unroll
+        for (int r = 0; r < 16; ++r)
+            o[ms * 16 + r] = (uint32_t)acc[ms][0][r] + ((uint32_t)acc[ms][1][r] << 8) + ((uint32_t)acc[ms][2][r] << 16) +
+                             ((uint32_t)acc[ms][3][r] << 24);
+    __syncthreads();
+#pragma unroll
+    for (int q = 0; q < 16 * MS; ++q) su[q * 64 + lane] = o[q];
+    __syncthreads();
+    constexpr int SHARE = 16 * MS / KSM_WAVES;
+    const int w = wt * KSM_WORDS + (lane & 31);
+#pragma unroll
+    for (int e = 0; e < SHARE; ++e) {
+        const int q = wave * SHARE + e;
+        uint32_t sum = 0;
+#pragma unroll
+        for (int v = 0; v < KSM_WAVES; ++v) sum += lds[v * BLOCK + q * 64 + lane];
+        const int r = q & 15, g = g0 + (q >> 4) * 32 + 8 * (r >> 2) + 4 * h + (r & 3);
+        if (g >= count || w >= p.ct_stride) continue;
+        const KsDesc d = descs[g];
+        uint32_t val = 0u - sum;
+        if (w == p.n) {
+            val += (uint32_t)u_buf[(size_t)d.u0 * p.u_stride + nin] + (uint32_t)d.add_b;
+            if (d.u1 >= 0) val += (uint32_t)u_buf[(size_t)d.u1 * p.u_stride + nin];
+        }
+        if (w > p.n) val = 0u;
+        pool[(size_t)d.dst_slot * p.ct_stride + w] = (int32_t)val;
+    }
+}
+
+bool launch_ksk_planes(hipStream_t s, const DevParams &p, const DevKey &key, uint8_t *image) {
+    const int nin = p.k * p.N;
+    if (!image || !ks_matrix_shape_ok(nin, p.ks_t, p.ks_basebit)) return false;
+    const long long total = (long long)(ks_matrix_image_bytes(nin, p.ct_stride) / 16);
+    hipLaunchKernelGGL(ksk_planes_kernel, dim3((unsigned)((total + 255) / 256)), dim3(256), 0, s, p, key,
+                       reinterpret_cast<uint4 *>(image), total);
+    return true;
+}
+
+bool launch_keyswitch_matrix(hipStream_t s, const DevParams &p, const uint8_t *image, const int32_t *u_buf,
+                             const KsDesc *descs, int count, int32_t *pool) {
+    const int nin = p.k * p.N;
+    if (!image || count <= 0 || !ks_matrix_shape_ok(nin, p.ks_t, p.ks_basebit) || (p.u_stride & 3)) return false;
+    const long long tiles = (count + KSM_GATES - 1) / KSM_GATES, wtiles = (p.ct_stride + KSM_WORDS - 1) / KSM_WORDS;
+    const long long per = (tiles * wtiles + 7) / 8;
+    if (per * 8 > 0x7fffffffLL) return false;
+    hipLaunchKernelGGL(keyswitch_matrix_kernel, dim3((unsigned)(per * 8)), dim3(KSM_WAVES * 64), 0, s, p,
+                       reinterpret_cast<const uint4 *>(image), u_buf, descs, count, pool, (int)tiles, (int)wtiles, (int)per);
+    return true;
+}
+
+}
diff --git a/peba1_amd/csrc/ks_matrix.hpp b/peba1_amd/csrc/ks_matrix.hpp
--- /dev/null
+++ b/peba1_amd/csrc/ks_matrix.hpp
@@ -0,0 +1,28 @@
+#pragma once
+#include "kernels.hpp"
+
+namespace tfhe_hip {
+
+__host__ __device__ inline void ks_byte_planes(uint32_t w, int8_t s[4]) {
+    uint32_t carry = 0;
+    for (int p = 0; p < 4; ++p) {
+        const uint32_t t = ((w >> (8 * p)) & 0xffu) + carry;
+        carry = t >= 128u ? 1u : 0u;
+        s[p] = (int8_t)(int)(t - (carry << 8));
+    }
+}
+
+constexpr int KSM_GATES = 64, KSM_WORDS = 32, KSM_WAVES = 8, KSM_CHUNK = 32;
+
+inline bool ks_matrix_shape_ok(int nin, int ks_t, int ks_basebit) {
+    return ks_t == 8 && ks_basebit == 2 && nin > 0 && nin % (KSM_WAVES * KSM_CHUNK) == 0;
+}
+inline size_t ks_matrix_image_bytes(int nin, int ct_stride) {
+    return (size_t)((ct_stride + KSM_WORDS - 1) / KSM_WORDS) * (size_t)nin * 4 * 64 * 16;
+}
+
+bool launch_ksk_planes(hipStream_t s, const DevParams &p, const DevKey &key, uint8_t *image);
+bool launch_keyswitch_matrix(hipStream_t s, const DevParams &p, const uint8_t *image, const int32_t *u_buf,
+                             const KsDesc *descs, int count, int32_t *pool);
+
+}
diff --git a/peba1_amd/csrc/launch_plan.hpp b/peba1_amd/csrc/launch_plan.hpp
--- a/peba1_amd/csrc/launch_plan.hpp
+++ b/peba1_amd/csrc/launch_plan.hpp
@@ -18,6 +18,8 @@
     int ks_split_ties = 0;
     int ks_tile = 16;
     int ks_index = 1;
+    int ks_matrix = 1;
+    int ks_matrix_min = 512;
 };
 
 inline void fill_form_ok(bool form_ok[BR_FORM_COUNT][3], int N, int l, int Bgbit) {
@@ -61,17 +63,20 @@
 
 inline int ks_threads(const KsShape &p) { return ((p.ct_stride / 4 + 63) / 64) * 64; }
 
-enum KsForm { KS_FORM_PERGATE = 0, KS_FORM_STRIP = 1, KS_FORM_INDEX = 2 };
+enum KsForm { KS_FORM_PERGATE = 0, KS_FORM_STRIP = 1, KS_FORM_INDEX = 2, KS_FORM_MATRIX = 3 };
+constexpr int KS_MATRIX_TILE = 64;
+constexpr int KS_MATRIX_SPAN = 256;
 struct KsPlan { int form; int tile; };
 
 inline int ks_tile_size(const LaunchTunings &t) { return (t.ks_tile > 16 && !t.ks_index) ? 16 : t.ks_tile; }
 
-inline KsPlan plan_ks(const LaunchTunings &t, int count, const KsShape &p) {
+inline KsPlan plan_ks(const LaunchTunings &t, int count, const KsShape &p, bool matrix = false) {
     const int tile = ks_tile_size(t), threads = ks_threads(p);
     const bool tiled = (tile == 16 || tile == 24 || tile == 32) && count >= 2 * tile && p.ks_t == 8 && p.ks_basebit == 2 &&
                        t.ks_max_splits > 1 && (p.nin + t.ks_max_splits - 1) / t.ks_max_splits <= 64 &&
                        (threads == 128 || threads == 192 || threads == 320);
     if (!tiled) return KsPlan{KS_FORM_PERGATE, 0};
+    if (matrix && t.ks_matrix && count >= t.ks_matrix_min && p.nin % KS_MATRIX_SPAN == 0) return KsPlan{KS_FORM_MATRIX, KS_MATRIX_TILE};
     return KsPlan{t.ks_index ? KS_FORM_INDEX : KS_FORM_STRIP, tile};
 }
 
@@ -146,7 +151,7 @@
     int n, N, k, l, Bgbit, ks_t, ks_basebit;
     int cus;
     int br_variant, br8_max_rotations, br_tail8, br_digit_table, ks_tile, ks_index, ks_max_splits, ks_target_blocks,
-        ks_split_ties;
+        ks_split_ties, ks_matrix, ks_matrix_min;
     int count;
     const int32_t *width;
     const double *us;
@@ -168,7 +173,8 @@
             e.ks_basebit == p.ks_basebit && e.cus == cus && e.br_variant == t.br_variant &&
             e.br8_max_rotations == t.br8_max_rotations && e.br_tail8 == t.br_tail8 && e.br_digit_table == t.br_digit_table &&
             e.ks_tile == t.ks_tile && e.ks_index == t.ks_index && e.ks_max_splits == t.ks_max_splits &&
-            e.ks_target_blocks == t.ks_target_blocks && e.ks_split_ties == t.ks_split_ties)
+            e.ks_target_blocks == t.ks_target_blocks && e.ks_split_ties == t.ks_split_ties && e.ks_matrix == t.ks_matrix &&
+            e.ks_matrix_min == t.ks_matrix_min)
             return LevelCost{e.width, e.us, e.count, 2 * e.cus};
     }
     return LevelCost{};
@@ -179,8 +185,9 @@
     return c.n ? level_cost_at(c, width) : -1.0;
 }
 
-inline size_t ks_partial_bytes(const LaunchTunings &t, int cu_count, int count, const KsShape &p) {
+inline size_t ks_partial_bytes(const LaunchTunings &t, int cu_count, int count, const KsShape &p, bool matrix = false) {
     size_t most = 0;
+    if (plan_ks(t, count, p, matrix).form == KS_FORM_MATRIX) return 0;
     const int chunk = ks_tiled(t, count, p) ? KS_CHUNK : count;
     for (int done = 0; done < count; done += chunk) {
         const int cnt = std::min(chunk, count - done), splits = ks_splits(t, cu_count, cnt, p);
diff --git a/peba1_amd/csrc/shim.cpp b/peba1_amd/csrc/shim.cpp
--- a/peba1_amd/csrc/shim.cpp
+++ b/peba1_amd/csrc/shim.cpp
@@ -826,6 +826,12 @@
         Engine::get().tunings.ks_max_splits = (int)value;
         return 0;
     }
+    if (name && std::strcmp(name, "ks_matrix") == 0) { Engine::get().tunings.ks_matrix = value != 0; return 0; }
+    if (name && std::strcmp(name, "ks_matrix_min") == 0) {
+        if (value < 1 || value > (1 << 30)) { set_error("ks_matrix_min must be in [1, 2^30]"); return -1; }
+        Engine::get().tunings.ks_matrix_min = (int)value;
+        return 0;
+    }
     if (name && std::strcmp(name, "br_digit_table") == 0) { Engine::get().tunings.br_digit_table = (int)value; return 0; }
     if (name && std::strcmp(name, "br8_max_rotations") == 0) { Engine::get().tunings.br8_max_rotations = (int)value; return 0; }
     if (name && std::strcmp(name, "br_tail8") == 0) { Engine::get().tunings.br_tail8 = (int)value; return 0; }
@@ -845,12 +851,17 @@
     auto g = recorder_lock();
     Engine::get().stats = TfheHipStats{};
     Engine::get().expand_stats = TfheHipExpandStats{};
+    Engine::get().ks_matrix_stats = TfheHipKsMatrixStats{};
     Engine::get().seeded_stats = TfheHipSeededStats{};
     Engine::get().seeded_lwe_stats = TfheHipSeededLweStats{};
 }
 void tfhe_hip_get_seeded_stats(TfheHipSeededStats *out) {
     auto g = recorder_lock();
     if (out) *out = Engine::get().seeded_stats;
+}
+void tfhe_hip_get_ks_matrix_stats(TfheHipKsMatrixStats *out) {
+    auto g = recorder_lock();
+    if (out) *out = Engine::get().ks_matrix_stats;
 }
 void tfhe_hip_get_expand_stats(TfheHipExpandStats *out) {
     auto g = recorder_lock();
diff --git a/peba1_amd/kernel_id.py b/peba1_amd/kernel_id.py
--- a/peba1_amd/kernel_id.py
+++ b/peba1_amd/kernel_id.py
@@ -3,7 +3,7 @@
 
 CSRC = os.path.join(os.path.dirname(os.path.abspath(__file__)), "csrc")
 KERNEL_FILES = ("kernels.hip", "kernels.hpp", "ntt_wave.hpp", "ntt_field.hpp", "br_forms.hpp", "ks_index_asm.inc", "br8_body.inc",
-                "build.sh")
+                "ks_matrix.hip", "ks_matrix.hpp", "build.sh")
 
 
 def kernels_sha16():
diff --git a/peba1_amd/lib.py b/peba1_amd/lib.py
--- a/peba1_amd/lib.py
+++ b/peba1_amd/lib.py
@@ -65,6 +65,10 @@
 
 class ExpandStats(C.Structure):
     _fields_ = [("expanded_keys", C.c_uint64), ("expand_launches", C.c_uint64)]
+
+
+class KsMatrixStats(C.Structure):
+    _fields_ = [("ks_matrix_launches", C.c_uint64)]
 
 
 class SeededStats(C.Structure):
@@ -208,6 +212,9 @@
     "tfhe_hip_kernel_lut_bootstrap_multi_woks": (C.c_int, [CK, I32P, C.c_int32, I32P, I32P, C.c_int32, I32P, I32P, C.c_int32,
                                                            I32P, I32P]),
     "tfhe_hip_kernel_keyswitch": (C.c_int, [CK, I32P, C.c_int32, I32P]),
+    "tfhe_hip_kernel_keyswitch_matrix": (C.c_int, [CK, I32P, C.c_int32, I32P]),
+    "tfhe_hip_test_ks_plan_form2": (C.c_int, [C.c_int32] * 5 + [I32P, C.c_int32, C.c_int32, C.c_int32, C.POINTER(C.c_int64)]),
+    "tfhe_hip_test_ks_byte_planes": (C.c_int, [U32P, C.c_int32, C.POINTER(C.c_int8)]),
     "tfhe_hip_new_packing_key": (C.c_void_p, [SK, C.c_int32, C.c_int32]),
     "tfhe_hip_new_packing_key_seeded": (C.c_void_p, [SK, C.c_int32, C.c_int32, C.c_uint64]),
     "tfhe_hip_new_packing_key_from_words": (C.c_void_p, [PS, C.c_int32, C.c_int32, I32P]),
@@ -244,6 +251,7 @@
     "tfhe_hip_test_key_image": (C.c_int64, [CK, C.c_int, I32P, C.c_int64]),
     "tfhe_hip_last_expand_ms": (C.c_double, []),
     "tfhe_hip_get_expand_stats": (None, [C.POINTER(ExpandStats)]),
+    "tfhe_hip_get_ks_matrix_stats": (None, [C.POINTER(KsMatrixStats)]),
     "tfhe_hip_get_seeded_stats": (None, [C.POINTER(SeededStats)]),
     "tfhe_hip_new_compressed_packing_key": (C.c_void_p, [SK, C.c_int32, C.c_int32]),
     "tfhe_hip_new_compressed_packing_key_seeded": (C.c_void_p, [SK, C.c_int32, C.c_int32, C.c_uint64, U32P]),
```

Result: faster. 112,000, median of 6 (+1.8%).
